# phuang1024/Starst3r

Hardware: AMD Instinct MI355X
Metric: 3DGS train iters/sec @ 1M Gaussians, 8x1080p views (higher is better)
Workload: dtype f32

## Files before the change

starst3r_amd/build.py:

```python
import concurrent.futures as cf
import os
import subprocess
import sys

HERE = os.path.dirname(os.path.abspath(__file__))
CSRC = os.path.join(HERE, "csrc")
OBJ = os.path.join(HERE, "_build")
LIB = os.path.join(HERE, "libst3r_hip.so")
HIPCC = os.environ.get("HIPCC", "/opt/rocm/bin/hipcc")

COMMON = ["--offload-arch=gfx950", "-O3", "-std=c++17", "-fPIC", "-fvisibility=hidden", "-munsafe-fp-atomics",
          "-Wall", "-Wno-unused-function", "-Wno-unused-result", "-DNDEBUG"] + os.environ.get("ST3R_DEFS", "").split()
PER_FILE = {
    "gs_project.hip": ["-ffp-contract=off"],
    "gs_isect.hip": ["-ffp-contract=off"],
    "recip_nn.hip": ["-mllvm", "-amdgpu-mfma-vgpr-form"],
}
NO_PACKED_F32 = ["-Xclang", "-target-feature", "-Xclang", "-packed-fp32-ops"]


def sources():
    return sorted(f for f in os.listdir(CSRC) if f.endswith(".hip"))


def _deps_mtime():
    hdrs = [os.path.join(CSRC, f) for f in os.listdir(CSRC) if f.endswith(".h")]
    hdrs.append(os.path.join(HERE, "..", "include", "st3r.h"))
    return max(os.path.getmtime(h) for h in hdrs)


def _compile(src, force, verbose):
    obj = os.path.join(OBJ, src.replace(".hip", ".o"))
    srcp = os.path.join(CSRC, src)
    if not force and os.path.exists(obj) and os.path.getmtime(obj) > max(os.path.getmtime(srcp), _deps_mtime()):
        return obj, False
    cmd = [HIPCC] + COMMON + NO_PACKED_F32 + PER_FILE.get(src, []) + ["-c", srcp, "-o", obj]
    if verbose:
        print(" ".join(cmd), flush=True)
    r = subprocess.run(cmd, capture_output=True, text=True)
    if r.returncode != 0:
        raise RuntimeError(f"hipcc failed for {src}:\n{r.stdout}\n{r.stderr}")
    noise = "is not a recognized feature for this target"
    err = "\n".join(l for l in r.stderr.splitlines() if l.strip() and noise not in l)
    if verbose and err:
        print(err)
    return obj, True


def build(force=False, verbose=False):
    os.makedirs(OBJ, exist_ok=True)
    srcs = sources()
    with cf.ThreadPoolExecutor(max_workers=min(8, len(srcs))) as ex:
        res = list(ex.map(lambda s: _compile(s, force, verbose), srcs))
    objs = [o for o, _ in res]
    if force or any(c for _, c in res) or not os.path.exists(LIB):
        cmd = [HIPCC, "--offload-arch=gfx950", "-shared", "-fPIC", "-o", LIB] + objs + ["-ldl"]
        if verbose:
            print(" ".join(cmd), flush=True)
        subprocess.check_call(cmd)
    return LIB


if __name__ == "__main__":
    print(build(force="--force" in sys.argv, verbose=("-v" in sys.argv or True)))
```

starst3r_amd/csrc/fused_step.hip:

```cpp
#include "radix_sort.h"
#include "stages.h"

int st3r_count_settle(st3r_ctx* ctx) {
    if (!ctx->count_pending) return ST3R_OK;
    HIP_TRY(hipEventSynchronize(ctx->count_event));
    ctx->count_pending = 0;
    const int64_t n = (int64_t)((int32_t*)(ctx->pinned + 8))[0];
    if (n < 0) {
        ctx->isect_hint = 0;
        ctx->view_chunks = (ctx->view_chunks > 0 ? ctx->view_chunks : 1) * 2;
        st3r_set_error("the previous step produced more than 2^31 tile intersections: its gradients were incomplete -- "
                       "repeat it (st3r_gs_train_fwd_bwd / st3r_gs_train_step now walk the views in %d chunks)",
                       ctx->view_chunks);
        return ST3R_ERR_CAPACITY;
    }
    if (n > ctx->count_cap) {
        ctx->isect_hint = 0;
        st3r_set_error("the previous step produced %lld tile intersections, more than the %lld its buffers were sized "
                       "for from the step before (+25 %%): its gradients were incomplete and st3r_adam_step / "
                       "st3r_gs_train_step did NOT apply them (the update is guarded on the device) -- repeat that step",
                       (long long)n, (long long)ctx->count_cap);
        return ST3R_ERR_CAPACITY;
    }
    ctx->isect_hint = n;
    return ST3R_OK;
}

struct FrontPlan {
    int tile_w, tile_h;
    bool key32;
    bool segments;
    int rect32;
    bool rectbase;
    uint32_t key_base;
    int l1_end_bit;
    int end_bit;
};
static const float k_near_plane = 0.01f, k_far_plane = 1e10f;
static FrontPlan front_plan(int C, int W, int H, int debug_flags, bool with_reg, bool records) {
    FrontPlan p;
    const int tile = 16;
    p.tile_w = (W + tile - 1) / tile; p.tile_h = (H + tile - 1) / tile;
    uint32_t near_bits, far_bits;
    memcpy(&near_bits, &k_near_plane, 4); memcpy(&far_bits, &k_far_plane, 4);
    p.key32 = (C <= 8) && (far_bits - near_bits < 0x1FFFFFFFu);
    p.key_base = p.key32 ? near_bits : 0u;
    p.rect32 = (p.tile_w <= 255 && p.tile_h <= 255 && !(debug_flags & 64)) ? 1 : 0;
    p.segments = p.key32 && with_reg && !records && !(debug_flags & 4);
    p.l1_end_bit = (p.key32 ? 29 : 32) + bit_length_u32((uint32_t)(C - 1));
    p.rectbase = p.tile_w <= 1023 && p.tile_h <= 1023 && !(debug_flags & 64);
    p.end_bit = bit_length_u32((uint32_t)((int64_t)C * p.tile_w * p.tile_h - 1));
    return p;
}

static int rasterize_front(st3r_ctx* ctx, hipStream_t s, const GsParams& g, const GsViews& v, double* reg_sums, int tight,
                           const float* records_in, bool allow_async, RasterOut* o, double* loss_sums = nullptr) {
    const int N = g.N, C = v.C, W = v.W, H = v.H;
    const int tile = 16;
    const FrontPlan fp = front_plan(C, W, H, ctx->debug_flags, reg_sums != nullptr, records_in != nullptr);
    const int tile_w = fp.tile_w, tile_h = fp.tile_h;
    const int64_t n_pairs = (int64_t)N * C;
    float* splats = const_cast<float*>(records_in);
    if (!records_in) {
        ARENA_GET(SLOT_SPLATS, float, n_pairs * ST3R_SPLAT_STRIDE, own);
        splats = own;
    }
    ARENA_GET(SLOT_CUM, int32_t, n_pairs, cum);
    ARENA_GET(SLOT_OFFSETS, int32_t, (int64_t)C * tile_w * tile_h + 1, offsets);
    const float near_plane = k_near_plane, far_plane = k_far_plane;
    const bool key32 = fp.key32;
    ARENA_GET(SLOT_DKEYS_A, uint64_t, n_pairs, dkeys_a);
    ARENA_GET(SLOT_DKEYS_B, uint64_t, n_pairs, dkeys_b);
    ARENA_GET(SLOT_DVALS_A, int32_t, n_pairs, dvals_a);
    ARENA_GET(SLOT_DVALS_B, int32_t, n_pairs, perm);
    const int rect32 = fp.rect32;
    ARENA_GET(SLOT_RECTS, uint64_t, rect32 ? (n_pairs + 1) / 2 : n_pairs, rects);
    int32_t* counts = nullptr;
    { int rc_ = st3r_counts_buffer(ctx, s, &counts); if (rc_) return rc_; }
    uint32_t* const krange = fp.segments ? (uint32_t*)(counts + 8) : nullptr;
    st3r_prof_begin(ctx, s, STG_PROJECT);
    const uint32_t key_base = fp.key_base;
    int rc = records_in
                 ? st3r_records_prepare_impl(s, N, C, splats, tile, tile_w, tile_h, tight, nullptr, dkeys_a, dvals_a,
                                             key_base, rects, rect32)
                 : st3r_project_impl(ctx, s, g, v, tile, 0.3f, near_plane, far_plane, 0.0f, splats, nullptr, reg_sums,
                                     dkeys_a, dvals_a, tight, key_base, rects, rect32, 1, loss_sums, 2 * C, krange);
    if (!rc && records_in && loss_sums) HIP_TRY(hipMemsetAsync(loss_sums, 0, sizeof(double) * 2 * (size_t)C, s));
    st3r_prof_end(ctx, s, STG_PROJECT);
    if (rc) return rc;
    st3r_prof_begin(ctx, s, STG_SORT_DEPTH);
    rc = krange ? st3r_radix_sort_u32_segments(ctx, s, N, C, (uint32_t*)dkeys_a, dvals_a, (uint32_t*)dkeys_b, perm, krange)
         : key32 ? st3r_radix_sort_u32(ctx, s, n_pairs, 0, fp.l1_end_bit, (uint32_t*)dkeys_a, dvals_a, (uint32_t*)dkeys_b, perm, nullptr)
                 : st3r_radix_sort_u64(ctx, s, n_pairs, 0, fp.l1_end_bit, dkeys_a, dvals_a, dkeys_b, perm);
    st3r_prof_end(ctx, s, STG_SORT_DEPTH);
    if (rc) return rc;
    int64_t n_isects = 0;
    st3r_prof_begin(ctx, s, STG_SCAN);
    uint64_t* rectbase = nullptr;
    if (fp.rectbase) {
        ARENA_GET(SLOT_RECTBASE, uint64_t, n_pairs, rb);
        rectbase = rb;
    }
    const int64_t sig = ((int64_t)N << 34) ^ ((int64_t)C << 26) ^ ((int64_t)W << 13) ^ (int64_t)H;
    const bool async = allow_async && ctx->isect_hint > 0 && ctx->hint_sig == sig;
    int32_t* total_dev = nullptr;
    rc = st3r_isect_scan_impl(ctx, s, n_pairs, nullptr, cum, nullptr, rects, rect32, rectbase, &total_dev,
                              async ? counts : nullptr, async ? (int32_t*)(ctx->pinned + 8) : nullptr);
    st3r_prof_end(ctx, s, STG_SCAN);
    if (rc) return rc;
    if (async) {
        if (!ctx->count_event) HIP_TRY(hipEventCreateWithFlags(&ctx->count_event, hipEventDisableTiming));
        HIP_TRY(hipEventRecord(ctx->count_event, s));
        n_isects = ctx->isect_hint + ctx->isect_hint / 4 + 1024;
        if (ctx->debug_flags & 8) n_isects = ctx->isect_hint / 2;
        if (n_isects > 2147483647LL) n_isects = 2147483647LL;
        ctx->count_pending = 1; ctx->count_cap = n_isects;
        o->n_visible = -1; o->n_isects_ref = -1;
    } else {
        HIP_TRY(hipMemcpyAsync(ctx->pinned, total_dev, sizeof(int32_t), hipMemcpyDeviceToHost, s));
        if (reg_sums) HIP_TRY(hipMemcpyAsync(ctx->pinned + 1, reg_sums + 2, 2 * sizeof(double), hipMemcpyDeviceToHost, s));
        HIP_TRY(hipStreamSynchronize(s));
        n_isects = (int64_t)((int32_t*)ctx->pinned)[0];
        if (n_isects < 0) {
            st3r_set_error("more than 2^31 tile intersections in one call: split the views over more calls / GPUs");
            return ST3R_SPLIT_VIEWS;
        }
        o->n_visible = reg_sums ? (int64_t)((double*)ctx->pinned)[1] : -1;
        o->n_isects_ref = reg_sums ? (int64_t)((double*)ctx->pinned)[2] : n_isects;
        if (allow_async) { ctx->isect_hint = n_isects; ctx->hint_sig = sig; }
    }
    ARENA_GET(SLOT_KEYS_A, uint32_t, n_isects, tkeys_a);
    ARENA_GET(SLOT_KEYS_B, uint32_t, n_isects, tkeys_b);
    ARENA_GET(SLOT_VALS_A, int32_t, n_isects, vals_a);
    ARENA_GET(SLOT_VALS_B, int32_t, n_isects, vals_b);
    o->n_records = async ? -1 : n_isects;
    const int64_t n_keys = (int64_t)C * tile_w * tile_h;
    const uint32_t* band_table = nullptr;
    const uint32_t* band_hist = nullptr;
    int n_bands = 0;
    if (n_isects > 0) {
        const int end_bit = fp.end_bit;
        const bool banded = st3r_sort_tile_banded(end_bit, ctx->debug_flags) != 0;
        const bool packed = banded && n_pairs <= (1 << 24) && !(ctx->debug_flags & 1024);
        n_bands = (int)((n_keys - 1) >> 8) + 1;
        st3r_prof_begin(ctx, s, STG_EMIT);
        rc = st3r_isect_emit_chain_impl(ctx, s, N, C, perm, rects, rect32, tile_w, tile_h, packed ? nullptr : tkeys_a, vals_a,
                                        n_isects, banded ? st3r_radix_sort_band_tile(n_isects) : 0, total_dev, &band_table);
        st3r_prof_end(ctx, s, STG_EMIT);
        if (rc) return rc;
        st3r_prof_begin(ctx, s, STG_SORT);
        rc = packed ? st3r_radix_sort_u32_banded_packed(ctx, s, n_isects, n_bands, band_table, (const uint32_t*)vals_a, vals_b,
                                                        &band_hist)
             : banded ? st3r_radix_sort_u32_banded(ctx, s, n_isects, n_bands, band_table, tkeys_a, vals_a, tkeys_b, vals_b)
                      : st3r_sort_tile_impl(ctx, s, n_isects, end_bit, tkeys_a, vals_a, tkeys_b, vals_b, total_dev);
        st3r_prof_end(ctx, s, STG_SORT);
        if (rc) return rc;
    }
    st3r_prof_begin(ctx, s, STG_OFFSETS);
    rc = band_hist ? st3r_radix_band_offsets(s, n_bands, band_table, band_hist, n_keys, offsets)
                   : st3r_isect_offsets32_impl(s, n_isects, tkeys_b, C, tile_w, tile_h, offsets, total_dev);
    st3r_prof_end(ctx, s, STG_OFFSETS);
    if (rc) return rc;
    o->C = C; o->W = W; o->H = H; o->tile_w = tile_w; o->tile_h = tile_h;
    o->splats = splats; o->offsets = offsets; o->flat = vals_b; o->cum = cum; o->rects = rect32 ? nullptr : rects;
    o->rectbase = rectbase;
    o->tight = tight; o->n_pairs = n_pairs;
    o->n_isects = n_isects;
    return ST3R_OK;
}

__global__ void k_finalize_loss(int C, const double* __restrict__ sums, const double* __restrict__ reg_sums,
                                double inv_px, double inv_cnt, double w_l1, double w_ssim, double reg_views,
                                double opac_k, double scale_k, float* __restrict__ loss_out,
                                const double* __restrict__ dsums, const double* __restrict__ dnorm, double depth_fac,
                                const double* __restrict__ wnorm, const double* __restrict__ asums,
                                const double* __restrict__ anorm, double alpha_fac) {
    if (threadIdx.x == 0 && blockIdx.x == 0) {
        double loss = 0;
        if (wnorm)
            for (int c = 0; c < C; ++c)
                loss += w_l1 * sums[2 * c] / (3.0 * fmax(wnorm[2 * c], 1.0)) +
                        w_ssim * (3.0 * wnorm[2 * c + 1] - sums[2 * c + 1]) / (3.0 * fmax(wnorm[2 * c + 1], 1.0));
        else
            for (int c = 0; c < C; ++c) loss += w_l1 * sums[2 * c] * inv_px + w_ssim * (1.0 - sums[2 * c + 1] * inv_cnt);
        loss += reg_views * (opac_k * reg_sums[0] + scale_k * reg_sums[1]);
        if (dsums)
            for (int c = 0; c < C; ++c) loss += depth_fac * dsums[c] / dnorm[c];
        if (asums)
            for (int c = 0; c < C; ++c) loss += alpha_fac * asums[c] / anorm[c];
        loss_out[0] = (float)loss;
    }
}

static int finalize_loss(hipStream_t s, int C, int H, int W, const double* sums, const double* reg_sums, float ssim_fac,
                         double reg_views, double opac_k, double scale_k, float* loss_out, const double* dp_sums,
                         const DepthPrior& dp, const LossWeight& lw, const double* at_sums = nullptr,
                         const AlphaTarget& at = AlphaTarget{}) {
    const int Hi = H - 10, Wi = W - 10;
    const double cnt = (Hi > 0 && Wi > 0) ? (double)Hi * Wi * 3 : 0.0;
    hipLaunchKernelGGL(k_finalize_loss, dim3(1), dim3(64), 0, s, C, sums, reg_sums, 1.0 / ((double)H * W * 3),
                       cnt > 0 ? 1.0 / cnt : 0.0, (double)(1.0f - ssim_fac), (double)ssim_fac, reg_views, opac_k, scale_k,
                       loss_out, dp_sums, dp.norm, (double)dp.fac, lw.weight ? lw.norm : nullptr, at_sums, at.norm,
                       (double)at.fac);
    LAUNCH_CHECK();
    return ST3R_OK;
}

struct LossFacs { float ssim, opac, scale; };

struct ViewBatch {
    GsViews v;
    const float* gt;
    double* sums;
    double* dp_sums;
    float* v_viewmats;
    bool exposure;
    bool weighted;
    bool background;
    double* at_sums;
    ViewBatch slice(int c0, int c1) const {
        return {v.slice(c0, c1), gt + (int64_t)c0 * v.H * v.W * 3, sums + 2 * c0, dp_sums ? dp_sums + c0 : nullptr,
                v_viewmats ? v_viewmats + 16 * c0 : nullptr, exposure, weighted, background,
                at_sums ? at_sums + c0 : nullptr};
    }
};

struct StepImages { float *rgb, *alpha; int32_t* last; float *v_rgb, *depth, *v_depth, *v_alpha, *exposed, *composite; };

static int step_images(st3r_ctx* ctx, const RasterOut& ro, bool with_depth, bool with_exposure, bool with_background,
                       bool with_v_alpha, StepImages* im) {
    const int64_t n_px = (int64_t)ro.C * ro.H * ro.W;
    ARENA_GET(SLOT_RGB, float, n_px * 3, rgb);
    ARENA_GET(SLOT_ALPHA, float, n_px, alpha);
    ARENA_GET(SLOT_LAST, int32_t, n_px, last);
    ARENA_GET(SLOT_VRENDER, float, n_px * 3, v_rgb);
    *im = StepImages{rgb, alpha, last, v_rgb, nullptr, nullptr, nullptr, nullptr, nullptr};
    if (with_exposure) {
        ARENA_GET(SLOT_EXPOSED, float, n_px * 3, exposed);
        im->exposed = exposed;
    }
    if (with_background) {
        ARENA_GET(SLOT_COMPOSITE, float, n_px * 3, composite);
        im->composite = composite;
    }
    if (with_depth) {
        ARENA_GET(SLOT_DEPTH, float, n_px, depth);
        ARENA_GET(SLOT_VDEPTH, float, n_px, v_depth);
        im->depth = depth; im->v_depth = v_depth;
    }
    if (with_depth || with_v_alpha) {
        ARENA_GET(SLOT_VALPHA, float, n_px, v_alpha);
        im->v_alpha = v_alpha;
    }
    return ST3R_OK;
}

static int forward_and_losses(st3r_ctx* ctx, hipStream_t s, const RasterOut& ro, const ViewBatch& b, float ssim_fac,
                              bool sums_cleared, const DepthPrior& dp, const ExposureReg& ex, const LossWeight& lw,
                              const StepImages& im, const Background& bg = Background{},
                              const AlphaTarget& at = AlphaTarget{}) {
    const bool eio = true;
    st3r_prof_begin(ctx, s, STG_BLEND_FWD);
    int rc = st3r_blend_fwd_impl(ctx, s, ro, im.rgb, im.alpha, im.last, true, eio);
    if (!rc && dp.prior) rc = st3r_blend_depth_fwd_impl(ctx, s, ro, im.last, im.depth, eio);
    st3r_prof_end(ctx, s, STG_BLEND_FWD);
    if (rc) return rc;
    st3r_prof_begin(ctx, s, STG_LOSS);
    const float* x = im.rgb;
    if (bg.colors) {
        rc = st3r_composite_fwd_impl(s, ro.C, ro.H, ro.W, im.rgb, im.alpha, bg.colors, im.composite);
        x = im.composite;
    }
    if (!rc && ex.exposure) rc = st3r_exposure_fwd_impl(s, ro.C, ro.H, ro.W, x, ex.exposure, im.exposed);
    if (!rc)
        rc = st3r_loss_impl(ctx, s, ro.C, ro.H, ro.W, ex.exposure ? im.exposed : x, b.gt, 1.0f - ssim_fac, ssim_fac,
                            b.sums, im.v_rgb, sums_cleared, lw);
    if (!rc && ex.exposure)
        rc = st3r_exposure_bwd_impl(ctx, s, ro.C, ro.H, ro.W, x, ex.exposure, im.v_rgb, im.v_rgb, ex.v_exposure);
    if (!rc && dp.prior)
        rc = st3r_depth_prior_loss_impl(ctx, s, ro.C, ro.H, ro.W, im.depth, im.alpha, dp.prior, dp.weight, dp.norm, 1, dp.fac,
                                        b.dp_sums, 1, im.v_depth, im.v_alpha);
    if (!rc && (bg.colors || at.target))
        rc = st3r_alpha_grad_impl(ctx, s, ro.C, ro.H, ro.W, im.alpha, bg.colors, bg.colors ? im.v_rgb : nullptr, at.target,
                                  at.weight, at.norm, 1, at.fac, dp.prior ? im.v_alpha : nullptr, b.at_sums, 1, im.v_alpha,
                                  nullptr);
    st3r_prof_end(ctx, s, STG_LOSS);
    return rc;
}

static int blend_backward(st3r_ctx* ctx, hipStream_t s, const RasterOut& ro, const StepImages& im, bool need_pairs,
                          st3r_vtile_ref* slots, float* v_pairs) {
    RasterOut rb = ro;
    if (ctx->debug_flags & 2) { rb.rects = nullptr; rb.rectbase = nullptr; }
    const bool eio = true;
    st3r_prof_begin(ctx, s, STG_BLEND_BWD);
    int rc = st3r_blend_bwd_impl(ctx, s, rb, im.alpha, im.last, im.v_rgb, im.v_alpha, nullptr, eio, slots);
    if (!rc && need_pairs) {
        ARENA_GET(SLOT_VSPLATS_D, float, ro.n_pairs * ST3R_SPLAT_STRIDE, v_pairs_d);
        rc = st3r_blend_depth_bwd_impl(ctx, s, rb, im.alpha, im.last, im.v_depth, v_pairs_d, eio);
        if (!rc) {
            if (slots->vtile) rc = st3r_gather_vtile_impl(s, ro.n_pairs, slots, v_pairs);
            else HIP_TRY(hipMemsetAsync(v_pairs, 0, sizeof(float) * ST3R_SPLAT_STRIDE * (size_t)ro.n_pairs, s));
        }
        if (!rc) rc = st3r_add_pairs_impl(s, ro.n_pairs, v_pairs, v_pairs_d);
    }
    st3r_prof_end(ctx, s, STG_BLEND_BWD);
    return rc;
}

static int project_backward(st3r_ctx* ctx, hipStream_t s, const GsParams& g, const GsViews& v, const RasterOut& ro,
                            const LossFacs& f, const float* v_pairs, const st3r_vtile_ref* slots, bool accumulate,
                            float* grads) {
    ctx->ranges_recorded = 0;
    if (!(ctx->n_ranges > 1 && ctx->comm_stream))
        return st3r_project_sh_bwd_impl(s, g, v, 0.3f, ro.splats, v_pairs, (float)v.C, f.opac, f.scale, grads, accumulate, 0,
                                        -1, false, slots);
    ARENA_GET(SLOT_GSTAGE, float, (int64_t)23 * g.N, gstage);
    const int K = ctx->n_ranges;
    for (int j = 0; j < K; ++j) {
        const int g0 = (int)((int64_t)g.N * j / K), g1 = (int)((int64_t)g.N * (j + 1) / K);
        int rc = st3r_project_sh_bwd_impl(s, g, v, 0.3f, ro.splats, v_pairs, (float)v.C, f.opac, f.scale, gstage, accumulate,
                                          g0, g1, true, slots);
        if (rc) return rc;
        HIP_TRY(hipEventRecord(ctx->ev_range_bwd[j], s));
    }
    ctx->ranges_recorded = K;
    return ST3R_OK;
}

static int pose_backward(st3r_ctx* ctx, hipStream_t s, const GsParams& g, const GsViews& v, const RasterOut& ro,
                         const float* v_pairs, float* v_viewmats) {
    return st3r_gs_viewmat_bwd(ctx, s, g.N, v.C, g.means, g.quats, g.scales, g.sh, g.sh_stride, v.viewmats, v.Ks, v.campos,
                               v.W, v.H, 0.3f, ro.splats, v_pairs, v_viewmats);
}

static int train_views(st3r_ctx* ctx, hipStream_t s, const GsParams& g, const ViewBatch& b, const LossFacs& f,
                       double* reg_sums, bool allow_async, bool accumulate, float* grads, RasterOut* ro_out) {
    const GsViews& v = b.v;
    DepthPrior dp{};
    int rc = b.dp_sums ? st3r_depth_prior_for(ctx, s, b.gt, v.C, v.H, v.W, &dp) : ST3R_OK;
    if (rc) return rc;
    ExposureReg ex{};
    if (b.exposure) st3r_exposure_for(ctx, b.gt, v.C, v.H, v.W, &ex);
    LossWeight lw{};
    if (b.weighted) rc = st3r_loss_weight_for(ctx, s, b.gt, v.C, v.H, v.W, &lw);
    if (rc) return rc;
    Background bg{};
    if (b.background) st3r_background_for(ctx, b.gt, v.C, v.H, v.W, &bg);
    AlphaTarget at{};
    if (b.at_sums) rc = st3r_alpha_target_for(ctx, s, b.gt, v.C, v.H, v.W, &at);
    if (rc) return rc;
    const bool need_pairs = dp.prior != nullptr;
    RasterOut& ro = *ro_out;
    rc = rasterize_front(ctx, s, g, v, reg_sums, 1, nullptr, allow_async, &ro, b.sums);
    if (rc) return rc;
    StepImages im;
    rc = step_images(ctx, ro, need_pairs, ex.exposure != nullptr, bg.colors != nullptr, bg.colors || at.target, &im);
    if (rc) return rc;
    float* const v_Ks = st3r_intrinsics_grad_for(ctx, b.gt, v.C, v.H, v.W);
    float* v_pairs = nullptr;
    if (need_pairs || b.v_viewmats || v_Ks) {
        ARENA_GET(SLOT_VSPLATS, float, ro.n_pairs * ST3R_SPLAT_STRIDE, vp);
        v_pairs = vp;
    }
    rc = forward_and_losses(ctx, s, ro, b, f.ssim, true, dp, ex, lw, im, bg, at);
    if (rc) return rc;
    st3r_vtile_ref slots{};
    rc = blend_backward(ctx, s, ro, im, need_pairs, &slots, v_pairs);
    if (rc) return rc;
    st3r_prof_begin(ctx, s, STG_PROJECT_BWD);
    rc = project_backward(ctx, s, g, v, ro, f, need_pairs ? v_pairs : nullptr, need_pairs ? nullptr : &slots, accumulate,
                          grads);
    if (!rc && need_pairs && b.v_viewmats) rc = pose_backward(ctx, s, g, v, ro, v_pairs, b.v_viewmats);
    if (!rc && need_pairs) rc = st3r_gs_depth_bwd(ctx, s, g.N, v.C, g.means, v.viewmats, ro.splats, v_pairs, grads, b.v_viewmats);
    st3r_prof_end(ctx, s, STG_PROJECT_BWD);
    if (!rc && !need_pairs && (b.v_viewmats || v_Ks)) {
        rc = st3r_gather_vtile_impl(s, ro.n_pairs, &slots, v_pairs);
        if (!rc && b.v_viewmats) rc = pose_backward(ctx, s, g, v, ro, v_pairs, b.v_viewmats);
    }
    if (!rc && v_Ks)
        rc = st3r_gs_intrinsics_bwd(ctx, s, g.N, v.C, g.means, g.quats, g.scales, v.viewmats, v.Ks, v.W, v.H, 0.3f,
                                    ro.splats, v_pairs, v_Ks);
    return rc;
}

static int train_chunks(st3r_ctx* ctx, hipStream_t s, const GsParams& g, const ViewBatch& all, const LossFacs& f,
                        double* reg_sums, double* reg_scratch, bool want_stats, float* grads, int* chunks, int64_t stats[3]) {
    const int C = all.v.C;
    for (;;) {
        int rc = ST3R_OK;
        stats[0] = stats[1] = stats[2] = 0;
        bool first = true;
        for (int k = 0; k < *chunks && !rc; ++k) {
            const int c0 = (int)((int64_t)k * C / *chunks), c1 = (int)((int64_t)(k + 1) * C / *chunks);
            if (c1 == c0) continue;
            RasterOut ro;
            rc = train_views(ctx, s, g, all.slice(c0, c1), f, first ? reg_sums : reg_scratch,
                             !want_stats && *chunks == 1 && !ctx->comm, !first, grads, &ro);
            if (!rc) { stats[0] += ro.n_visible; stats[1] += ro.n_records; stats[2] += ro.n_isects_ref; }
            first = false;
        }
        if (rc == ST3R_SPLIT_VIEWS && *chunks < C) {
            *chunks = *chunks * 2 < C ? *chunks * 2 : C;
            continue;
        }
        return rc == ST3R_SPLIT_VIEWS ? ST3R_ERR_INVALID : rc;
    }
}

int st3r_train_fwd_bwd_impl(st3r_ctx* ctx, hipStream_t s, const GsParams& g, const GsViews& v, const float* gt_images,
                            float ssim_fac, float opac_fac, float scale_fac, float* grads, float* loss_out,
                            int64_t* stats_host, float* v_viewmats) {
    const int N = g.N, C = v.C;
    ARG_CHECK(ctx && N > 0 && C > 0 && C <= ST3R_MAX_VIEWS && v.W > 0 && v.H > 0 && g.sh_stride >= 12);
    ARG_CHECK((int64_t)N * C < 2147483647LL);
    ARG_CHECK(g.means && g.quats && g.scales && g.opacities && g.sh && v.viewmats && v.Ks && v.campos && gt_images && grads &&
              loss_out);
    ARENA_GET(SLOT_SMALL, double, 2 * (size_t)C + 12, small);
    double* sums = small;
    double* reg_sums = small + 2 * C;
    double* dp_sums = nullptr;
    DepthPrior dp;
    int rc = st3r_depth_prior_for(ctx, s, gt_images, C, v.H, v.W, &dp);
    if (rc) return rc;
    if (dp.prior) {
        if (ctx->comm) {
            st3r_set_error("a depth prior is registered and a communicator is attached -- the depth term is not "
                           "supported in view-sharded training (clear it with st3r_ctx_set_depth_prior(ctx, NULL, ...))");
            return ST3R_ERR_INVALID;
        }
        ARENA_GET(SLOT_DPRIOR_SUMS, double, (size_t)C, ds);
        dp_sums = ds;
    }
    ExposureReg ex;
    st3r_exposure_for(ctx, gt_images, C, v.H, v.W, &ex);
    if (ex.exposure && ctx->comm) {
        st3r_set_error("exposures are registered and a communicator is attached -- per-view exposures are not supported "
                       "in view-sharded training (clear them with st3r_ctx_set_exposure(ctx, NULL, ...))");
        return ST3R_ERR_INVALID;
    }
    if (ctx->comm && st3r_intrinsics_grad_for(ctx, gt_images, C, v.H, v.W)) {
        st3r_set_error("an intrinsics gradient is registered and a communicator is attached -- intrinsics refinement is "
                       "not supported in view-sharded training (clear it with st3r_ctx_set_intrinsics_grad(ctx, NULL, ...))");
        return ST3R_ERR_INVALID;
    }
    LossWeight lw;
    rc = st3r_loss_weight_for(ctx, s, gt_images, C, v.H, v.W, &lw);
    if (rc) return rc;
    if (lw.weight && ctx->comm) {
        st3r_set_error("loss weights are registered and a communicator is attached -- per-pixel loss weights are not "
                       "supported in view-sharded training (clear them with st3r_ctx_set_loss_weight(ctx, NULL, ...))");
        return ST3R_ERR_INVALID;
    }
    Background bg;
    st3r_background_for(ctx, gt_images, C, v.H, v.W, &bg);
    if (bg.colors && ctx->comm) {
        st3r_set_error("backgrounds are registered and a communicator is attached -- backgrounds are not supported in "
                       "view-sharded training (clear them with st3r_ctx_set_background(ctx, NULL, ...))");
        return ST3R_ERR_INVALID;
    }
    double* at_sums = nullptr;
    AlphaTarget at;
    rc = st3r_alpha_target_for(ctx, s, gt_images, C, v.H, v.W, &at);
    if (rc) return rc;
    if (at.target) {
        if (ctx->comm) {
            st3r_set_error("alpha targets are registered and a communicator is attached -- alpha supervision is not "
                           "supported in view-sharded training (clear them with st3r_ctx_set_alpha_target(ctx, NULL, ...))");
            return ST3R_ERR_INVALID;
        }
        ARENA_GET(SLOT_ATARGET_SUMS, double, (size_t)C, as);
        at_sums = as;
    }
    st3r_prof_next_step(ctx);
    rc = st3r_count_settle(ctx);
    if (rc) return rc;
    int chunks = ctx->view_chunks > 0 ? ctx->view_chunks : 1;
    if ((ctx->debug_flags & 32) && chunks < 2) chunks = 2;
    if (chunks > C) chunks = C;
    int64_t stats[3];
    rc = train_chunks(ctx, s, g, ViewBatch{v, gt_images, sums, dp_sums, v_viewmats, ex.exposure != nullptr, lw.weight != nullptr,
                                           bg.colors != nullptr, at_sums},
                      LossFacs{ssim_fac, opac_fac, scale_fac},
                      reg_sums, reg_sums + 4, stats_host != nullptr, grads, &chunks, stats);
    if (rc) return rc;
    if (chunks > 1) ctx->view_chunks = chunks;
    rc = finalize_loss(s, C, v.H, v.W, sums, reg_sums, ssim_fac, (double)C, (double)opac_fac / N,
                       (double)scale_fac / (3.0 * N), loss_out, dp_sums, dp, lw, at_sums, at);
    if (rc) return rc;
    if (stats_host) {
        stats_host[0] = stats[0]; stats_host[1] = stats[1]; stats_host[2] = st3r_ctx_arena_bytes(ctx);
        stats_host[3] = stats[2];
    }
    return ST3R_OK;
}

ST3R_EXPORT int st3r_gs_train_fwd_bwd(st3r_ctx* ctx, void* stream, int N, int C, const float* means,
                                      const float* quats, const float* scales, const float* opacities,
                                      const float* sh, int sh_stride, const float* viewmats, const float* Ks,
                                      const float* campos, const float* gt_images, int width, int height,
                                      float ssim_fac, float opac_fac, float scale_fac, float* grads,
                                      float* loss_out, int64_t* stats_host) {
    return st3r_train_fwd_bwd_impl(ctx, (hipStream_t)stream, GsParams{N, means, quats, scales, opacities, sh, sh_stride},
                                   GsViews{C, width, height, viewmats, Ks, campos}, gt_images, ssim_fac, opac_fac,
                                   scale_fac, grads, loss_out, stats_host, nullptr);
}

ST3R_EXPORT int st3r_gs_raster_train(st3r_ctx* ctx, void* stream, int N, int C, const float* records,
                                     const float* gt_images, int width, int height, float ssim_fac,
                                     float* v_records, float* loss_out, int64_t* stats_host) {
    ARG_CHECK(ctx && N > 0 && C > 0 && width > 0 && height > 0 && records && gt_images && v_records && loss_out);
    ARG_CHECK(C <= ST3R_MAX_VIEWS && (int64_t)N * C < 2147483647LL);
    hipStream_t s = (hipStream_t)stream;
    ARENA_GET(SLOT_SMALL, double, 2 * (size_t)C + 8, sums);
    double* reg_sums = sums + 2 * C;
    const ViewBatch b{GsViews{C, width, height}, gt_images, sums, nullptr, nullptr, false, false, false, nullptr};
    HIP_TRY(hipMemsetAsync(reg_sums, 0, sizeof(double) * 4, s));
    st3r_prof_next_step(ctx);
    RasterOut ro;
    int rc = st3r_count_settle(ctx);
    if (rc) return rc;
    rc = rasterize_front(ctx, s, GsParams{N}, b.v, nullptr, 1, records, stats_host == nullptr, &ro);
    if (rc == ST3R_SPLIT_VIEWS) rc = ST3R_ERR_INVALID;
    if (rc) return rc;
    StepImages im;
    rc = step_images(ctx, ro, false, false, false, false, &im);
    if (rc) return rc;
    rc = forward_and_losses(ctx, s, ro, b, ssim_fac, false, DepthPrior{}, ExposureReg{}, LossWeight{}, im);
    if (rc) return rc;
    st3r_prof_begin(ctx, s, STG_BLEND_BWD);
    rc = st3r_blend_bwd_impl(ctx, s, ro, im.alpha, im.last, im.v_rgb, nullptr, v_records, true, nullptr);
    st3r_prof_end(ctx, s, STG_BLEND_BWD);
    if (rc) return rc;
    rc = finalize_loss(s, C, height, width, sums, reg_sums, ssim_fac, 0.0, 0.0, 0.0, loss_out, nullptr, DepthPrior{},
                       LossWeight{});
    if (rc) return rc;
    if (stats_host) {
        stats_host[0] = -1; stats_host[1] = ro.n_records; stats_host[2] = st3r_ctx_arena_bytes(ctx); stats_host[3] = -1;
    }
    return ST3R_OK;
}

ST3R_EXPORT int st3r_gs_render(st3r_ctx* ctx, void* stream, int N, int C, const float* means, const float* quats,
                               const float* scales, const float* opacities, const float* sh, int sh_stride,
                               const float* viewmats, const float* Ks, const float* campos, int width, int height,
                               float* rgb, float* alpha, int64_t* stats_host) {
    ARG_CHECK(ctx && N > 0 && C > 0 && width > 0 && height > 0 && sh_stride >= 12);
    ARG_CHECK(C <= ST3R_MAX_VIEWS && (int64_t)N * C < 2147483647LL);
    ARG_CHECK(means && quats && scales && opacities && sh && viewmats && Ks && campos && rgb && alpha);
    hipStream_t s = (hipStream_t)stream;
    RasterOut ro;
    int rc = st3r_count_settle(ctx);
    if (rc) return rc;
    rc = rasterize_front(ctx, s, GsParams{N, means, quats, scales, opacities, sh, sh_stride},
                         GsViews{C, width, height, viewmats, Ks, campos}, nullptr, 0, nullptr, false, &ro);
    if (rc == ST3R_SPLIT_VIEWS) rc = ST3R_ERR_INVALID;
    if (rc) return rc;
    ARENA_GET(SLOT_LAST, int32_t, (int64_t)C * height * width, last);
    rc = st3r_blend_fwd_impl(ctx, s, ro, rgb, alpha, last, false, true);
    if (rc) return rc;
    if (stats_host) {
        stats_host[0] = -1; stats_host[1] = ro.n_records; stats_host[2] = st3r_ctx_arena_bytes(ctx); stats_host[3] = 0;
    }
    return ST3R_OK;
}

ST3R_EXPORT int st3r_front_plan(int N, int C, int width, int height, int debug_flags, int training, int records,
                                int64_t n_records, int64_t* out, int n_out) {
    ARG_CHECK(N > 0 && C > 0 && C <= ST3R_MAX_VIEWS && width > 0 && height > 0 && n_records >= 0 && out &&
              n_out >= ST3R_FRONT_PLAN_WORDS && !(training && records));
    const FrontPlan fp = front_plan(C, width, height, debug_flags, training != 0, records != 0);
    const int64_t n_pairs = (int64_t)N * C;
    for (int i = 0; i < n_out; ++i) out[i] = 0;
    out[0] = fp.rect32; out[1] = fp.rectbase; out[2] = fp.key32; out[3] = fp.segments;
    out[4] = st3r_scan_tiles(n_pairs);
    int bpc, grid, self_base;
    st3r_emit_grid(N, C, &bpc, &grid, &self_base);
    out[5] = bpc; out[6] = grid; out[7] = self_base;
    int64_t sh[8];
    if (fp.segments) st3r_radix_sort_shape(4, n_pairs, N, C, 0, 0, sh);
    else st3r_radix_sort_shape(fp.key32 ? 4 : 8, n_pairs, 0, 0, 0, fp.l1_end_bit, sh);
    out[8] = sh[0]; out[9] = sh[1]; out[10] = sh[2]; out[11] = sh[3]; out[12] = sh[4];
    out[25] = sh[5];
    out[fp.key32 ? 26 : 28] = sh[6]; out[fp.key32 ? 27 : 29] = sh[7];
    st3r_radix_sort_shape(fp.key32 ? 8 : 4, 1, 0, 0, 0, 8, sh);
    out[fp.key32 ? 28 : 26] = sh[6]; out[fp.key32 ? 29 : 27] = sh[7];
    out[13] = st3r_sort_tile_end_bit(fp.end_bit);
    if (n_records > 0) {
        st3r_radix_sort_shape(4, n_records, 0, 0, 0, (int)out[13], sh);
        out[14] = sh[0]; out[15] = sh[1]; out[16] = sh[2]; out[17] = sh[4];
    }
    if (st3r_sort_tile_banded(fp.end_bit, debug_flags)) {
        out[18] = 1;
        out[19] = (((int64_t)C * fp.tile_w * fp.tile_h - 1) >> 8) + 1;
        if (n_records > 0) out[30] = n_records / st3r_radix_sort_band_tile(n_records) + out[19];
    }
    int64_t k[5];
    st3r_isect_constants(k);
    for (int i = 0; i < 5; ++i) out[20 + i] = k[i];
    return ST3R_OK;
}
```

starst3r_amd/csrc/gs_intrinsics.hip:

```cpp
#include "per_view.h"
#include "project_common.h"

__global__ __launch_bounds__(256) void k_intrinsics_bwd_part(
    int N, const float* __restrict__ means, const float* __restrict__ quats, const float* __restrict__ scales,
    const float* __restrict__ viewmats, const float* __restrict__ Ks, int W, int H, const float4* __restrict__ splats,
    const float4* __restrict__ v_splats, double* __restrict__ part) {
    __shared__ double red[4 * 4];
    const int c = blockIdx.y;
    const int g = blockIdx.x * blockDim.x + threadIdx.x;
    float v_fx = 0.f, v_fy = 0.f, v_cx = 0.f, v_cy = 0.f;
    const int64_t pid = (int64_t)c * N + g;
    if (g < N && __float_as_int(splats[pid * 3 + 2].z) > 0) {
        const float4 r0 = splats[pid * 3 + 0], r1 = splats[pid * 3 + 1];
        const float4 g0 = v_splats[pid * 3 + 0], g1 = v_splats[pid * 3 + 1];
        const float* V = viewmats + 16 * c;
        const float R[9] = {V[0], V[1], V[2], V[4], V[5], V[6], V[8], V[9], V[10]};
        const float* K = Ks + 9 * c;
        const float fx = K[0], fy = K[4], cx = K[2], cy = K[5];
        const float tan_fovx = 0.5f * (float)W / fx, tan_fovy = 0.5f * (float)H / fy;
        const float lim_xp = ((float)W - cx) / fx + 0.3f * tan_fovx, lim_xn = cx / fx + 0.3f * tan_fovx;
        const float lim_yp = ((float)H - cy) / fy + 0.3f * tan_fovy, lim_yn = cy / fy + 0.3f * tan_fovy;
        const float mx = means[3 * g], my = means[3 * g + 1], mz = means[3 * g + 2];
        float qw = quats[4 * g], qx = quats[4 * g + 1], qy = quats[4 * g + 2], qz = quats[4 * g + 3];
        const float sc[3] = {scales[3 * g], scales[3 * g + 1], scales[3 * g + 2]};
        const float inv_norm = 1.0f / sqrtf(((qw * qw + qx * qx) + qy * qy) + qz * qz);
        qw *= inv_norm; qx *= inv_norm; qy *= inv_norm; qz *= inv_norm;
        float cov[6];
        {
            float x2 = qx * qx, y2 = qy * qy, z2 = qz * qz, xy = qx * qy, xz = qx * qz, yz = qy * qz;
            float wx = qw * qx, wy = qw * qy, wz = qw * qz;
            const float Rq[9] = {1.0f - 2.0f * (y2 + z2), 2.0f * (xy - wz), 2.0f * (xz + wy),
                                 2.0f * (xy + wz), 1.0f - 2.0f * (x2 + z2), 2.0f * (yz - wx),
                                 2.0f * (xz - wy), 2.0f * (yz + wx), 1.0f - 2.0f * (x2 + y2)};
            float M[9];
#pragma unroll
            for (int i = 0; i < 3; ++i)
#pragma unroll
                for (int j = 0; j < 3; ++j) M[i * 3 + j] = Rq[i * 3 + j] * sc[j];
            cov[0] = M[0] * M[0] + M[1] * M[1] + M[2] * M[2];
            cov[1] = M[0] * M[3] + M[1] * M[4] + M[2] * M[5];
            cov[2] = M[0] * M[6] + M[1] * M[7] + M[2] * M[8];
            cov[3] = M[3] * M[3] + M[4] * M[4] + M[5] * M[5];
            cov[4] = M[3] * M[6] + M[4] * M[7] + M[5] * M[8];
            cov[5] = M[6] * M[6] + M[7] * M[7] + M[8] * M[8];
        }
        const float x = R[0] * mx + R[1] * my + R[2] * mz + V[3];
        const float y = R[3] * mx + R[4] * my + R[5] * mz + V[7];
        const float z = R[6] * mx + R[7] * my + R[8] * mz + V[11];
        float T[9];
#pragma unroll
        for (int i = 0; i < 3; ++i) {
            T[i * 3 + 0] = R[i * 3] * cov[0] + R[i * 3 + 1] * cov[1] + R[i * 3 + 2] * cov[2];
            T[i * 3 + 1] = R[i * 3] * cov[1] + R[i * 3 + 1] * cov[3] + R[i * 3 + 2] * cov[4];
            T[i * 3 + 2] = R[i * 3] * cov[2] + R[i * 3 + 1] * cov[4] + R[i * 3 + 2] * cov[5];
        }
        const Sym3 S = {T[0] * R[0] + T[1] * R[1] + T[2] * R[2], T[0] * R[3] + T[1] * R[4] + T[2] * R[5],
                        T[0] * R[6] + T[1] * R[7] + T[2] * R[8], T[3] * R[3] + T[4] * R[4] + T[5] * R[5],
                        T[3] * R[6] + T[4] * R[7] + T[5] * R[8], T[6] * R[6] + T[7] * R[7] + T[8] * R[8]};
        const float rz = 1.0f / z, rz2 = rz * rz;
        const float xr = x * rz, yr = y * rz;
        const bool x_in = (xr <= lim_xp) && (xr >= -lim_xn);
        const bool y_in = (yr <= lim_yp) && (yr >= -lim_yn);
        const float tx = z * fminf(lim_xp, fmaxf(-lim_xn, xr));
        const float ty = z * fminf(lim_yp, fmaxf(-lim_yn, yr));
        const float a = fx * rz, cj = -fx * tx * rz2, b = fy * rz, d = -fy * ty * rz2;
        Sym3 vS;
        float vJ00, vJ02, vJ11, vJ12;
        conic_chain(r0, r1, g0, g1, a, cj, b, d, S, vS, vJ00, vJ02, vJ11, vJ12);
        const float vm2x = g0.x, vm2y = g0.y;
        v_fx = vm2x * xr + vJ00 * rz;
        v_fy = vm2y * yr + vJ11 * rz;
        v_cx = vm2x; v_cy = vm2y;
        if (x_in) v_fx += -x * rz2 * vJ02;
        else v_cx += vJ02 * rz;
        if (y_in) v_fy += -y * rz2 * vJ12;
        else v_cy += vJ12 * rz;
    }
    double v[4] = {(double)v_fx, (double)v_fy, (double)v_cx, (double)v_cy};
    const double t = block_sum_fixed(v, red);
    if (threadIdx.x < 4) part[((int64_t)c * gridDim.x + blockIdx.x) * 4 + threadIdx.x] = t;
}

ST3R_EXPORT int st3r_gs_intrinsics_bwd(st3r_ctx* ctx, void* stream, int N, int C, const float* means, const float* quats,
                                       const float* scales, const float* viewmats, const float* Ks, int width, int height,
                                       float eps2d, const float* splats, const float* v_splats, float* v_Ks) {
    ARG_CHECK(ctx && N >= 0 && C > 0 && C <= ST3R_MAX_VIEWS && width > 0 && height > 0);
    ARG_CHECK(means && quats && scales && viewmats && Ks && splats && v_splats && v_Ks);
    (void)eps2d;
    hipStream_t s = (hipStream_t)stream;
    const int nb = ceil_div(N, 256);
    double* part = nullptr;
    if (nb > 0) {
        ARENA_GET(SLOT_KGRAD_PART, double, 4 * (size_t)nb * C, p);
        part = p;
        hipLaunchKernelGGL(k_intrinsics_bwd_part, dim3(nb, C), dim3(256), 0, s, N, means, quats, scales, viewmats, Ks,
                           width, height, (const float4*)splats, (const float4*)v_splats, part);
        LAUNCH_CHECK();
    }
    return stream_finish<4>(s, C, nb, (const double*)part, v_Ks, 4, 0);
}

float* st3r_intrinsics_grad_for(st3r_ctx* ctx, const float* gt, int C, int H, int W) {
    const int64_t c0 = view_reg_first(ctx->kg, gt, C, H, W);
    return c0 < 0 ? nullptr : ctx->kg_v_Ks + 4 * c0;
}

ST3R_EXPORT int st3r_ctx_set_intrinsics_grad(st3r_ctx* ctx, const float* gt, float* v_Ks, int C, int height, int width) {
    ARG_CHECK(ctx);
    const bool on = gt && v_Ks;
    int rc = view_reg_set(&ctx->kg, on, gt, C, height, width);
    if (rc) return rc;
    ctx->kg_v_Ks = on ? v_Ks : nullptr;
    return ST3R_OK;
}

__global__ __launch_bounds__(64) void k_intrinsics_adam(int C, PerViewAdamK k, float* __restrict__ Ks,
                                                        const float* __restrict__ v_Ks, float* __restrict__ k_m,
                                                        float* __restrict__ k_v, double W, double H, int mode) {
    const int c = per_view_adam_view(k, C);
    if (c < 0) return;
    float* K = Ks + 9 * c;
    const float* G = v_Ks + 4 * c;
    float* m = k_m + 4 * c;
    float* v = k_v + 4 * c;
    const double fx = (double)K[0], fy = (double)K[4];
    const double g0 = fx * (double)G[0], g1 = fy * (double)G[1];
    if (mode & 1) {
        const double e = exp(per_view_adam_delta<false>(k, m[0], g0 + g1, v[0]));
        K[0] = (float)(fx * e); K[4] = (float)(fy * e);
    } else {
        K[0] = (float)(fx * exp(per_view_adam_delta<false>(k, m[0], g0, v[0])));
        K[4] = (float)(fy * exp(per_view_adam_delta<false>(k, m[1], g1, v[1])));
    }
    if (mode & 2) {
        K[2] = (float)((double)K[2] + W * per_view_adam_delta<false>(k, m[2], W * (double)G[2], v[2]));
        K[5] = (float)((double)K[5] + H * per_view_adam_delta<false>(k, m[3], H * (double)G[3], v[3]));
    }
}

ST3R_EXPORT int st3r_intrinsics_adam_step(st3r_ctx* ctx, void* stream, int C, float* Ks, const float* v_Ks, float* k_m,
                                          float* k_v, double lr, double beta1, double beta2, double eps, int step,
                                          const float* mask, int width, int height, int mode) {
    ARG_CHECK(ctx && C > 0 && step >= 1 && beta1 >= 0.0 && beta1 < 1.0 && beta2 >= 0.0 && beta2 < 1.0);
    ARG_CHECK(Ks && v_Ks && k_m && k_v && width > 0 && height > 0 && mode >= 0 && mode <= 3);
    return per_view_adam_launch(ctx, (hipStream_t)stream, k_intrinsics_adam, C, lr, beta1, beta2, eps, step, mask, Ks, v_Ks,
                                k_m, k_v, (double)width, (double)height, mode);
}
```

starst3r_amd/csrc/gs_pose_bwd.hip:

```cpp
#include "per_view.h"
#include "project_common.h"

#define POSE_VALS 15

__device__ __forceinline__ void block_sum_pose(double (&v)[POSE_VALS], double* red) {
    const double sum = block_sum_fixed(v, red);
    if (threadIdx.x < POSE_VALS) red[4 * POSE_VALS + threadIdx.x] = sum;
    __syncthreads();
    if (threadIdx.x < POSE_VALS) red[threadIdx.x] = red[4 * POSE_VALS + threadIdx.x];
    __syncthreads();
}

__global__ __launch_bounds__(256) void k_viewmat_bwd_part(
    int N, const float* __restrict__ means, const float* __restrict__ quats, const float* __restrict__ scales,
    const float* __restrict__ sh, int sh_stride, const float* __restrict__ viewmats, const float* __restrict__ Ks,
    const float* __restrict__ campos, int W, int H, const float4* __restrict__ splats,
    const float4* __restrict__ v_splats, double* __restrict__ part) {
    __shared__ double red[5 * POSE_VALS];
    const int c = blockIdx.y;
    const int g = blockIdx.x * blockDim.x + threadIdx.x;
    float acc[POSE_VALS];
#pragma unroll
    for (int k = 0; k < POSE_VALS; ++k) acc[k] = 0.f;
    const int64_t pid = (int64_t)c * N + g;
    if (g < N && __float_as_int(splats[pid * 3 + 2].z) > 0) {
        const float4 r0 = splats[pid * 3 + 0], r1 = splats[pid * 3 + 1], r2 = splats[pid * 3 + 2];
        const float4 g0 = v_splats[pid * 3 + 0], g1 = v_splats[pid * 3 + 1], g2 = v_splats[pid * 3 + 2];
        const float* V = viewmats + 16 * c;
        const float R[9] = {V[0], V[1], V[2], V[4], V[5], V[6], V[8], V[9], V[10]};
        const float* K = Ks + 9 * c;
        const float fx = K[0], fy = K[4], cx = K[2], cy = K[5];
        const float tan_fovx = 0.5f * (float)W / fx, tan_fovy = 0.5f * (float)H / fy;
        const float lim_xp = ((float)W - cx) / fx + 0.3f * tan_fovx, lim_xn = cx / fx + 0.3f * tan_fovx;
        const float lim_yp = ((float)H - cy) / fy + 0.3f * tan_fovy, lim_yn = cy / fy + 0.3f * tan_fovy;
        const float mx = means[3 * g], my = means[3 * g + 1], mz = means[3 * g + 2];
        float qw = quats[4 * g], qx = quats[4 * g + 1], qy = quats[4 * g + 2], qz = quats[4 * g + 3];
        const float sc[3] = {scales[3 * g], scales[3 * g + 1], scales[3 * g + 2]};
        float k[12];
        const float* kp = sh + (int64_t)g * sh_stride;
#pragma unroll
        for (int i = 0; i < 12; ++i) k[i] = kp[i];
        const float inv_norm = 1.0f / sqrtf(((qw * qw + qx * qx) + qy * qy) + qz * qz);
        qw *= inv_norm; qx *= inv_norm; qy *= inv_norm; qz *= inv_norm;
        float cov[6];
        {
            float x2 = qx * qx, y2 = qy * qy, z2 = qz * qz, xy = qx * qy, xz = qx * qz, yz = qy * qz;
            float wx = qw * qx, wy = qw * qy, wz = qw * qz;
            const float Rq[9] = {1.0f - 2.0f * (y2 + z2), 2.0f * (xy - wz), 2.0f * (xz + wy),
                                 2.0f * (xy + wz), 1.0f - 2.0f * (x2 + z2), 2.0f * (yz - wx),
                                 2.0f * (xz - wy), 2.0f * (yz + wx), 1.0f - 2.0f * (x2 + y2)};
            float M[9];
#pragma unroll
            for (int i = 0; i < 3; ++i)
#pragma unroll
                for (int j = 0; j < 3; ++j) M[i * 3 + j] = Rq[i * 3 + j] * sc[j];
            cov[0] = M[0] * M[0] + M[1] * M[1] + M[2] * M[2];
            cov[1] = M[0] * M[3] + M[1] * M[4] + M[2] * M[5];
            cov[2] = M[0] * M[6] + M[1] * M[7] + M[2] * M[8];
            cov[3] = M[3] * M[3] + M[4] * M[4] + M[5] * M[5];
            cov[4] = M[3] * M[6] + M[4] * M[7] + M[5] * M[8];
            cov[5] = M[6] * M[6] + M[7] * M[7] + M[8] * M[8];
        }
        {
            float dx = mx - campos[3 * c], dy = my - campos[3 * c + 1], dz = mz - campos[3 * c + 2];
            float nrm = sqrtf(dx * dx + dy * dy + dz * dz);
            float inrm = 1.0f / nrm;
            float ux = dx * inrm, uy = dy * inrm, uz = dz * inrm;
            const float vcol[3] = {g1.z, g1.w, g2.x};
            const float colf[3] = {r1.z, r1.w, r2.x};
            float vdx = 0.f, vdy = 0.f, vdz = 0.f;
#pragma unroll
            for (int ch = 0; ch < 3; ++ch) {
                float pre = SH_C0 * k[ch] + SH_C1 * ((-uy * k[3 + ch] + uz * k[6 + ch]) - ux * k[9 + ch]) + 0.5f;
                float vc = (colf[ch] > 0.0f || pre >= 0.0f) ? vcol[ch] : 0.0f;
                vdx += -SH_C1 * k[9 + ch] * vc;
                vdy += -SH_C1 * k[3 + ch] * vc;
                vdz += SH_C1 * k[6 + ch] * vc;
            }
            float dotp = vdx * ux + vdy * uy + vdz * uz;
            acc[12] = -((vdx - dotp * ux) * inrm);
            acc[13] = -((vdy - dotp * uy) * inrm);
            acc[14] = -((vdz - dotp * uz) * inrm);
        }
        const float x = R[0] * mx + R[1] * my + R[2] * mz + V[3];
        const float y = R[3] * mx + R[4] * my + R[5] * mz + V[7];
        const float z = R[6] * mx + R[7] * my + R[8] * mz + V[11];
        float T[9];
#pragma unroll
        for (int i = 0; i < 3; ++i) {
            T[i * 3 + 0] = R[i * 3] * cov[0] + R[i * 3 + 1] * cov[1] + R[i * 3 + 2] * cov[2];
            T[i * 3 + 1] = R[i * 3] * cov[1] + R[i * 3 + 1] * cov[3] + R[i * 3 + 2] * cov[4];
            T[i * 3 + 2] = R[i * 3] * cov[2] + R[i * 3 + 1] * cov[4] + R[i * 3 + 2] * cov[5];
        }
        const float S00 = T[0] * R[0] + T[1] * R[1] + T[2] * R[2];
        const float S01 = T[0] * R[3] + T[1] * R[4] + T[2] * R[5];
        const float S02 = T[0] * R[6] + T[1] * R[7] + T[2] * R[8];
        const float S11 = T[3] * R[3] + T[4] * R[4] + T[5] * R[5];
        const float S12 = T[3] * R[6] + T[4] * R[7] + T[5] * R[8];
        const float S22 = T[6] * R[6] + T[7] * R[7] + T[8] * R[8];
        const float rz = 1.0f / z, rz2 = rz * rz, rz3 = rz2 * rz;
        const float xr = x * rz, yr = y * rz;
        const bool x_in = (xr <= lim_xp) && (xr >= -lim_xn);
        const bool y_in = (yr <= lim_yp) && (yr >= -lim_yn);
        const float tx = z * fminf(lim_xp, fmaxf(-lim_xn, xr));
        const float ty = z * fminf(lim_yp, fmaxf(-lim_yn, yr));
        const float a = fx * rz, cj = -fx * tx * rz2, b = fy * rz, d = -fy * ty * rz2;
        const Sym3 S = {S00, S01, S02, S11, S12, S22};
        Sym3 vS;
        float vJ00, vJ02, vJ11, vJ12;
        conic_chain(r0, r1, g0, g1, a, cj, b, d, S, vS, vJ00, vJ02, vJ11, vJ12);
        const float vm2x = g0.x, vm2y = g0.y;
        float vpx = fx * rz * vm2x;
        float vpy = fy * rz * vm2y;
        float vpz = -(fx * x * vm2x + fy * y * vm2y) * rz2;
        vpz += -fx * rz2 * vJ00 - fy * rz2 * vJ11;
        if (x_in) { vpx += -fx * rz2 * vJ02; vpz += 2.0f * fx * x * rz3 * vJ02; }
        else { vpz += fx * tx * rz3 * vJ02; }
        if (y_in) { vpy += -fy * rz2 * vJ12; vpz += 2.0f * fy * y * rz3 * vJ12; }
        else { vpz += fy * ty * rz3 * vJ12; }
        const float vSm[9] = {vS.xx, vS.xy, vS.xz, vS.xy, vS.yy, vS.yz, vS.xz, vS.yz, vS.zz};
        const float vp[3] = {vpx, vpy, vpz}, m[3] = {mx, my, mz};
#pragma unroll
        for (int i = 0; i < 3; ++i) {
#pragma unroll
            for (int j = 0; j < 3; ++j)
                acc[i * 3 + j] = vp[i] * m[j] +
                                 2.0f * (vSm[i * 3] * T[j] + vSm[i * 3 + 1] * T[3 + j] + vSm[i * 3 + 2] * T[6 + j]);
            acc[9 + i] = vp[i];
        }
    }
    double v[POSE_VALS];
#pragma unroll
    for (int k2 = 0; k2 < POSE_VALS; ++k2) v[k2] = (double)acc[k2];
    block_sum_pose(v, red);
    if (threadIdx.x < POSE_VALS)
        part[((int64_t)c * gridDim.x + blockIdx.x) * POSE_VALS + threadIdx.x] = red[threadIdx.x];
}

__global__ __launch_bounds__(256) void k_viewmat_bwd_finish(int n_part, const float* __restrict__ viewmats,
                                                           const double* __restrict__ part,
                                                           float* __restrict__ v_viewmats) {
    __shared__ double red[5 * POSE_VALS];
    const int c = blockIdx.x;
    double v[POSE_VALS];
#pragma unroll
    for (int k = 0; k < POSE_VALS; ++k) v[k] = 0.0;
    const double* pc = part + (int64_t)c * n_part * POSE_VALS;
    for (int b = threadIdx.x; b < n_part; b += blockDim.x) {
#pragma unroll
        for (int k = 0; k < POSE_VALS; ++k) v[k] += pc[(int64_t)b * POSE_VALS + k];
    }
    block_sum_pose(v, red);
    if (threadIdx.x >= 16) return;
    double a[16];
    const float* Vf = viewmats + 16 * c;
#pragma unroll
    for (int i = 0; i < 16; ++i) a[i] = (double)Vf[i];
    const double s0 = a[0] * a[5] - a[4] * a[1], s1 = a[0] * a[6] - a[4] * a[2], s2 = a[0] * a[7] - a[4] * a[3];
    const double s3 = a[1] * a[6] - a[5] * a[2], s4 = a[1] * a[7] - a[5] * a[3], s5 = a[2] * a[7] - a[6] * a[3];
    const double c5 = a[10] * a[15] - a[14] * a[11], c4 = a[9] * a[15] - a[13] * a[11], c3 = a[9] * a[14] - a[13] * a[10];
    const double c2 = a[8] * a[15] - a[12] * a[11], c1 = a[8] * a[14] - a[12] * a[10], c0 = a[8] * a[13] - a[12] * a[9];
    const double idet = 1.0 / (s0 * c5 - s1 * c4 + s2 * c3 + s3 * c2 - s4 * c1 + s5 * c0);
    double inv[16];
    inv[0] = (a[5] * c5 - a[6] * c4 + a[7] * c3) * idet;
    inv[1] = (-a[1] * c5 + a[2] * c4 - a[3] * c3) * idet;
    inv[2] = (a[13] * s5 - a[14] * s4 + a[15] * s3) * idet;
    inv[3] = (-a[9] * s5 + a[10] * s4 - a[11] * s3) * idet;
    inv[4] = (-a[4] * c5 + a[6] * c2 - a[7] * c1) * idet;
    inv[5] = (a[0] * c5 - a[2] * c2 + a[3] * c1) * idet;
    inv[6] = (-a[12] * s5 + a[14] * s2 - a[15] * s1) * idet;
    inv[7] = (a[8] * s5 - a[10] * s2 + a[11] * s1) * idet;
    inv[8] = (a[4] * c4 - a[5] * c2 + a[7] * c0) * idet;
    inv[9] = (-a[0] * c4 + a[1] * c2 - a[3] * c0) * idet;
    inv[10] = (a[12] * s4 - a[13] * s2 + a[15] * s0) * idet;
    inv[11] = (-a[8] * s4 + a[9] * s2 - a[11] * s0) * idet;
    inv[12] = (-a[4] * c3 + a[5] * c1 - a[6] * c0) * idet;
    inv[13] = (a[0] * c3 - a[1] * c1 + a[2] * c0) * idet;
    inv[14] = (-a[12] * s3 + a[13] * s1 - a[14] * s0) * idet;
    inv[15] = (a[8] * s3 - a[9] * s1 + a[10] * s0) * idet;
    const int i = threadIdx.x >> 2, j = threadIdx.x & 3;
    const double u = inv[i] * red[12] + inv[4 + i] * red[13] + inv[8 + i] * red[14];
    const double w = inv[4 * j + 3];
    const double base = i == 3 ? 0.0 : (j == 3 ? red[9 + i] : red[i * 3 + j]);
    v_viewmats[16 * c + threadIdx.x] = (float)(base - u * w);
}

ST3R_EXPORT int st3r_gs_viewmat_bwd(st3r_ctx* ctx, void* stream, int N, int C, const float* means, const float* quats,
                                    const float* scales, const float* sh, int sh_stride, const float* viewmats,
                                    const float* Ks, const float* campos, int width, int height, float eps2d,
                                    const float* splats, const float* v_splats, float* v_viewmats) {
    ARG_CHECK(ctx && N >= 0 && C > 0 && C <= ST3R_MAX_VIEWS && sh_stride >= 12 && width > 0 && height > 0);
    ARG_CHECK(means && quats && scales && sh && viewmats && Ks && campos && splats && v_splats && v_viewmats);
    (void)eps2d;
    hipStream_t s = (hipStream_t)stream;
    const int nb = ceil_div(N, 256);
    double* part = nullptr;
    if (nb > 0) {
        ARENA_GET(SLOT_POSE_PART, double, POSE_VALS * (size_t)nb * C, p);
        part = p;
        hipLaunchKernelGGL(k_viewmat_bwd_part, dim3(nb, C), dim3(256), 0, s, N, means, quats, scales, sh, sh_stride,
                           viewmats, Ks, campos, width, height, (const float4*)splats, (const float4*)v_splats, part);
        LAUNCH_CHECK();
    }
    hipLaunchKernelGGL(k_viewmat_bwd_finish, dim3(C), dim3(256), 0, s, nb, viewmats, (const double*)part, v_viewmats);
    LAUNCH_CHECK();
    return ST3R_OK;
}
```

starst3r_amd/csrc/gs_project.hip:

```cpp
#include "stages.h"
#include "tile_rect.h"
#include "project_common.h"

__device__ __forceinline__ float dot3f(float a0, float a1, float a2, float b0, float b1, float b2) {
    return (a0 * b0 + a1 * b1) + a2 * b2;
}

__global__ __launch_bounds__(256) void k_project_sh_fwd(
    int N, int C, const float* __restrict__ means, const float* __restrict__ quats,
    const float* __restrict__ scales, const float* __restrict__ opacities, const float* __restrict__ sh,
    int sh_stride, const float* __restrict__ viewmats, const float* __restrict__ Ks,
    const float* __restrict__ campos, int W, int H, int tile_size, int tile_w, int tile_h, float eps2d,
    float near_plane, float far_plane, float radius_clip, float4* __restrict__ splats,
    int32_t* __restrict__ tiles_per_gauss, double* __restrict__ reg_part,
    uint64_t* __restrict__ depth_keys, int32_t* __restrict__ depth_vals, int tight, uint32_t key_base,
    void* __restrict__ rects, int rect32, uint32_t* __restrict__ krange_part) {
    extern __shared__ float cam[];
    __shared__ float red[8];
    for (int c = threadIdx.x; c < C; c += blockDim.x) {
        float* o = cam + c * CAM_STRIDE;
        const float* V = viewmats + 16 * c;
        for (int k = 0; k < 12; ++k) o[k] = V[k];
        const float* K = Ks + 9 * c;
        float fx = K[0], fy = K[4], cx = K[2], cy = K[5];
        o[12] = fx; o[13] = fy; o[14] = cx; o[15] = cy;
        float tan_fovx = 0.5f * (float)W / fx;
        float tan_fovy = 0.5f * (float)H / fy;
        o[16] = ((float)W - cx) / fx + 0.3f * tan_fovx;
        o[17] = cx / fx + 0.3f * tan_fovx;
        o[18] = ((float)H - cy) / fy + 0.3f * tan_fovy;
        o[19] = cy / fy + 0.3f * tan_fovy;
        o[20] = campos[3 * c]; o[21] = campos[3 * c + 1]; o[22] = campos[3 * c + 2];
    }
    __syncthreads();

    const int g = blockIdx.x * blockDim.x + threadIdx.x;
    const bool active = g < N;
    float mx = 0, my = 0, mz = 0, opac = 0;
    float cov0 = 0, cov1 = 0, cov2 = 0, cov3 = 0, cov4 = 0, cov5 = 0;
    float k[12];
    float reg_o = 0.f, reg_s = 0.f;
    if (active) {
        mx = means[3 * g]; my = means[3 * g + 1]; mz = means[3 * g + 2];
        opac = opacities[g];
        float qw = quats[4 * g], qx = quats[4 * g + 1], qy = quats[4 * g + 2], qz = quats[4 * g + 3];
        float s0 = scales[3 * g], s1 = scales[3 * g + 1], s2 = scales[3 * g + 2];
        const float* kp = sh + (int64_t)g * sh_stride;
#pragma unroll
        for (int i = 0; i < 12; ++i) k[i] = kp[i];
        float n2 = ((qw * qw + qx * qx) + qy * qy) + qz * qz;
        float inv = 1.0f / sqrtf(n2);
        qw *= inv; qx *= inv; qy *= inv; qz *= inv;
        float x2 = qx * qx, y2 = qy * qy, z2 = qz * qz;
        float xy = qx * qy, xz = qx * qz, yz = qy * qz;
        float wx = qw * qx, wy = qw * qy, wz = qw * qz;
        float m0 = (1.0f - 2.0f * (y2 + z2)) * s0, m1 = (2.0f * (xy - wz)) * s1, m2 = (2.0f * (xz + wy)) * s2;
        float m3 = (2.0f * (xy + wz)) * s0, m4 = (1.0f - 2.0f * (x2 + z2)) * s1, m5 = (2.0f * (yz - wx)) * s2;
        float m6 = (2.0f * (xz - wy)) * s0, m7 = (2.0f * (yz + wx)) * s1, m8 = (1.0f - 2.0f * (x2 + y2)) * s2;
        cov0 = dot3f(m0, m1, m2, m0, m1, m2);
        cov1 = dot3f(m0, m1, m2, m3, m4, m5);
        cov2 = dot3f(m0, m1, m2, m6, m7, m8);
        cov3 = dot3f(m3, m4, m5, m3, m4, m5);
        cov4 = dot3f(m3, m4, m5, m6, m7, m8);
        cov5 = dot3f(m6, m7, m8, m6, m7, m8);
        if (reg_part) {
            reg_o = 1.0f / (1.0f + __expf(-opac));
            reg_s = (__expf(s0) + __expf(s1)) + __expf(s2);
        }
    }
    if (reg_part) {
        for (int off = 32; off > 0; off >>= 1) {
            reg_o += __shfl_down(reg_o, off);
            reg_s += __shfl_down(reg_s, off);
        }
        int w = threadIdx.x >> 6;
        if ((threadIdx.x & 63) == 0) { red[w] = reg_o; red[4 + w] = reg_s; }
        __syncthreads();
        if (threadIdx.x == 0) {
            reg_part[4 * blockIdx.x + 0] = (double)((red[0] + red[1]) + (red[2] + red[3]));
            reg_part[4 * blockIdx.x + 1] = (double)((red[4] + red[5]) + (red[6] + red[7]));
        }
    }
    int n_vis = 0, n_ref = 0;
    uint32_t kmin = 0xFFFFFFFFu, kmax = 0u;
    for (int c = 0; active && c < C; ++c) {
        const float* o = cam + c * CAM_STRIDE;
        const float R00 = o[0], R01 = o[1], R02 = o[2], t0 = o[3];
        const float R10 = o[4], R11 = o[5], R12 = o[6], t1 = o[7];
        const float R20 = o[8], R21 = o[9], R22 = o[10], t2 = o[11];
        const int64_t pid = (int64_t)c * N + g;
        float x = dot3f(R00, R01, R02, mx, my, mz) + t0;
        float y = dot3f(R10, R11, R12, mx, my, mz) + t1;
        float z = dot3f(R20, R21, R22, mx, my, mz) + t2;
        bool valid = !(z < near_plane || z > far_plane);
        float m2x = 0, m2y = 0, ca = 0, cb = 0, cc = 0, radius = 0;
        if (valid) {
            float T0 = dot3f(R00, R01, R02, cov0, cov1, cov2), T1 = dot3f(R00, R01, R02, cov1, cov3, cov4),
                  T2 = dot3f(R00, R01, R02, cov2, cov4, cov5);
            float T3 = dot3f(R10, R11, R12, cov0, cov1, cov2), T4 = dot3f(R10, R11, R12, cov1, cov3, cov4),
                  T5 = dot3f(R10, R11, R12, cov2, cov4, cov5);
            float T6 = dot3f(R20, R21, R22, cov0, cov1, cov2), T7 = dot3f(R20, R21, R22, cov1, cov3, cov4),
                  T8 = dot3f(R20, R21, R22, cov2, cov4, cov5);
            float c0 = dot3f(T0, T1, T2, R00, R01, R02);
            float c1 = dot3f(T0, T1, T2, R10, R11, R12);
            float c2 = dot3f(T0, T1, T2, R20, R21, R22);
            float c3 = dot3f(T3, T4, T5, R10, R11, R12);
            float c4 = dot3f(T3, T4, T5, R20, R21, R22);
            float c5 = dot3f(T6, T7, T8, R20, R21, R22);
            const float fx = o[12], fy = o[13], cx = o[14], cy = o[15];
            float rz = 1.0f / z;
            float rz2 = rz * rz;
            float xr = x * rz, yr = y * rz;
            float tx = z * fminf(o[16], fmaxf(-o[17], xr));
            float ty = z * fminf(o[18], fmaxf(-o[19], yr));
            float a = fx * rz, cj = -(fx * tx) * rz2;
            float b = fy * rz, d = -(fy * ty) * rz2;
            float t0x = a * c0 + cj * c2;
            float t0y = a * c1 + cj * c4;
            float t0z = a * c2 + cj * c5;
            float t1y = b * c3 + d * c4;
            float t1z = b * c4 + d * c5;
            float c00 = t0x * a + t0z * cj;
            float c01 = t0y * b + t0z * d;
            float c11 = t1y * b + t1z * d;
            m2x = (fx * x) * rz + cx;
            m2y = (fy * y) * rz + cy;
            c00 += eps2d; c11 += eps2d;
            float det = c00 * c11 - c01 * c01;
            if (det <= 0.0f) valid = false;
            else {
                float inv_det = 1.0f / det;
                ca = c11 * inv_det; cb = -c01 * inv_det; cc = c00 * inv_det;
                float bb = 0.5f * (c00 + c11);
                float v1 = bb + sqrtf(fmaxf(0.01f, bb * bb - det));
                radius = ceilf(3.0f * sqrtf(v1));
                if (radius <= radius_clip) valid = false;
                else if (m2x + radius <= 0.0f || m2x - radius >= (float)W || m2y + radius <= 0.0f ||
                         m2y - radius >= (float)H)
                    valid = false;
            }
        }
        float4 r0 = make_float4(0, 0, 0, 0), r1 = r0, r2 = r0;
        int ntiles = 0;
        TileRect tr = {0, 0, 0, 0};
        if (valid) {
            float dx = mx - o[20], dy = my - o[21], dz = mz - o[22];
            float inorm = 1.0f / sqrtf((dx * dx + dy * dy) + dz * dz);
            dx *= inorm; dy *= inorm; dz *= inorm;
            float col[3];
#pragma unroll
            for (int ch = 0; ch < 3; ++ch) {
                float r = SH_C0 * k[ch];
                r = r + SH_C1 * ((-dy * k[3 + ch] + dz * k[6 + ch]) - dx * k[9 + ch]);
                r = r + 0.5f;
                col[ch] = r < 0.0f ? 0.0f : r;
            }
            tr = ref_tile_rect(m2x, m2y, radius, tile_size, tile_w, tile_h);
            n_ref += (tr.y1 - tr.y0) * (tr.x1 - tr.x0);
            if (tight) tr = tight_tile_rect(tr, m2x, m2y, opac, ca, cb, cc);
            ntiles = (tr.y1 - tr.y0) * (tr.x1 - tr.x0);
            r0 = make_float4(m2x, m2y, opac, ca);
            r1 = make_float4(cb, cc, col[0], col[1]);
            r2 = make_float4(col[2], z, __int_as_float((int)radius), 0.0f);
        }
        splats[pid * 3 + 0] = r0;
        splats[pid * 3 + 1] = r1;
        splats[pid * 3 + 2] = r2;
        if (tiles_per_gauss) tiles_per_gauss[pid] = ntiles;
        if (rects) rect_store(rects, rect32, pid, tr);
        if (depth_keys) {
            const uint32_t dbits = valid ? (uint32_t)__float_as_int(z) : 0xFFFFFFFFu;
            if (key_base) {
                const uint32_t kk = valid ? dbits - key_base : 0x1FFFFFFFu;
                reinterpret_cast<uint32_t*>(depth_keys)[pid] = (krange_part ? 0u : ((uint32_t)c << 29)) | kk;
                if (valid) { kmin = min(kmin, kk); kmax = max(kmax, kk); }
            } else
                depth_keys[pid] = ((uint64_t)c << 32) | dbits;
            if (!krange_part) depth_vals[pid] = (int32_t)pid;
        }
        n_vis += valid ? 1 : 0;
    }
    if (krange_part) {
        for (int off = 32; off > 0; off >>= 1) { kmin = min(kmin, (uint32_t)__shfl_down((int)kmin, off)); kmax = max(kmax, (uint32_t)__shfl_down((int)kmax, off)); }
        __shared__ uint32_t redk[8];
        const int w = threadIdx.x >> 6;
        if ((threadIdx.x & 63) == 0) { redk[w] = kmin; redk[4 + w] = kmax; }
        __syncthreads();
        if (threadIdx.x == 0) {
            krange_part[2 * blockIdx.x + 0] = min(min(redk[0], redk[1]), min(redk[2], redk[3]));
            krange_part[2 * blockIdx.x + 1] = max(max(redk[4], redk[5]), max(redk[6], redk[7]));
        }
    }
    if (reg_part) {
        for (int off = 32; off > 0; off >>= 1) { n_vis += __shfl_down(n_vis, off); n_ref += __shfl_down(n_ref, off); }
        __shared__ int redi[8];
        const int w = threadIdx.x >> 6;
        if ((threadIdx.x & 63) == 0) { redi[w] = n_vis; redi[4 + w] = n_ref; }
        __syncthreads();
        if (threadIdx.x == 0) {
            reg_part[4 * blockIdx.x + 2] = (double)((redi[0] + redi[1]) + (redi[2] + redi[3]));
            reg_part[4 * blockIdx.x + 3] = (double)((redi[4] + redi[5]) + (redi[6] + redi[7]));
        }
    }
}

__global__ __launch_bounds__(256) void k_reg_reduce(int n_blocks, const double* __restrict__ reg_part,
                                                    double* __restrict__ reg_sums, int overwrite,
                                                    double* __restrict__ zero_ptr, int zero_n,
                                                    const uint32_t* __restrict__ krange_part,
                                                    uint32_t* __restrict__ krange) {
    for (int i = threadIdx.x; i < zero_n; i += 256) zero_ptr[i] = 0.0;
    if (krange_part) {
        __shared__ uint32_t shk[2][256];
        uint32_t lo = 0xFFFFFFFFu, hi = 0u;
        for (int b = threadIdx.x; b < n_blocks; b += 256) { lo = min(lo, krange_part[2 * b]); hi = max(hi, krange_part[2 * b + 1]); }
        shk[0][threadIdx.x] = lo; shk[1][threadIdx.x] = hi;
        __syncthreads();
        for (int off = 128; off > 0; off >>= 1) {
            if (threadIdx.x < off) {
                shk[0][threadIdx.x] = min(shk[0][threadIdx.x], shk[0][threadIdx.x + off]);
                shk[1][threadIdx.x] = max(shk[1][threadIdx.x], shk[1][threadIdx.x + off]);
            }
            __syncthreads();
        }
        if (threadIdx.x == 0) {
            lo = shk[0][0]; hi = shk[1][0];
            if (hi < lo) { lo = 0u; hi = 0u; }
            const uint32_t top = hi - lo + 1u;
            krange[0] = lo; krange[1] = top;
            krange[2] = top < (1u << 8) ? 1u : top < (1u << 16) ? 2u : top < (1u << 24) ? 3u : 4u;
        }
        __syncthreads();
    }
    __shared__ double sh[4][256];
    double acc[4] = {0, 0, 0, 0};
    for (int b = threadIdx.x; b < n_blocks; b += 256)
        for (int k = 0; k < 4; ++k) acc[k] += reg_part[4 * b + k];
    for (int k = 0; k < 4; ++k) sh[k][threadIdx.x] = acc[k];
    __syncthreads();
    for (int off = 128; off > 0; off >>= 1) {
        if (threadIdx.x < off)
            for (int k = 0; k < 4; ++k) sh[k][threadIdx.x] += sh[k][threadIdx.x + off];
        __syncthreads();
    }
    if (threadIdx.x < 4) reg_sums[threadIdx.x] = (overwrite ? 0.0 : reg_sums[threadIdx.x]) + sh[threadIdx.x][0];
}

int st3r_project_impl(st3r_ctx* ctx, hipStream_t s, const GsParams& g, const GsViews& v, int tile_size, float eps2d,
                      float near_plane, float far_plane, float radius_clip, float* splats, int32_t* tiles_per_gauss,
                      double* reg_sums, uint64_t* depth_keys, int32_t* depth_vals, int tight, uint32_t key_base, void* rects,
                      int rect32, int reg_overwrite, double* zero_ptr, int zero_n, uint32_t* krange) {
    const int N = g.N, C = v.C, width = v.W, height = v.H;
    if (N == 0) {
        if (reg_sums && reg_overwrite) HIP_TRY(hipMemsetAsync(reg_sums, 0, sizeof(double) * 4, s));
        if (zero_ptr && zero_n > 0) HIP_TRY(hipMemsetAsync(zero_ptr, 0, sizeof(double) * (size_t)zero_n, s));
        return ST3R_OK;
    }
    int tile_w = (width + tile_size - 1) / tile_size, tile_h = (height + tile_size - 1) / tile_size;
    dim3 grid(ceil_div(N, 256)), block(256);
    size_t shmem = (size_t)C * CAM_STRIDE * sizeof(float);
    double* reg_part = nullptr;
    if (reg_sums) {
        ARENA_GET(SLOT_REG_PART, double, 4 * (size_t)grid.x, p);
        reg_part = p;
    }
    uint32_t* krange_part = nullptr;
    if (krange && reg_sums) {
        ARENA_GET(SLOT_KRANGE_PART, uint32_t, 2 * (size_t)grid.x, p);
        krange_part = p;
    }
    hipLaunchKernelGGL(k_project_sh_fwd, grid, block, shmem, s, N, C, g.means, g.quats, g.scales, g.opacities, g.sh,
                       g.sh_stride, v.viewmats, v.Ks, v.campos, width, height, tile_size, tile_w, tile_h, eps2d, near_plane, far_plane,
                       radius_clip, (float4*)splats, tiles_per_gauss, reg_part, depth_keys, depth_vals, tight, key_base,
                       rects, rect32, krange_part);
    if (reg_sums)
        hipLaunchKernelGGL(k_reg_reduce, dim3(1), dim3(256), 0, s, (int)grid.x, reg_part, reg_sums, reg_overwrite, zero_ptr,
                           zero_ptr ? zero_n : 0, (const uint32_t*)krange_part, krange);
    else if (zero_ptr && zero_n > 0)
        HIP_TRY(hipMemsetAsync(zero_ptr, 0, sizeof(double) * (size_t)zero_n, s));
    LAUNCH_CHECK();
    return ST3R_OK;
}

ST3R_EXPORT int st3r_gs_project_sh(st3r_ctx* ctx, void* stream, int N, int C, const float* means,
                                   const float* quats, const float* scales, const float* opacities,
                                   const float* sh, int sh_stride, const float* viewmats, const float* Ks,
                                   const float* campos, int width, int height, int tile_size, float eps2d,
                                   float near_plane, float far_plane, float radius_clip, float* splats,
                                   int32_t* tiles_per_gauss, double* reg_sums) {
    ARG_CHECK(ctx && N >= 0 && C > 0 && C <= ST3R_MAX_VIEWS && sh_stride >= 12 && width > 0 && height > 0 && tile_size > 0);
    ARG_CHECK(means && quats && scales && opacities && sh && viewmats && Ks && campos && splats && tiles_per_gauss);
    return st3r_project_impl(ctx, (hipStream_t)stream, GsParams{N, means, quats, scales, opacities, sh, sh_stride},
                             GsViews{C, width, height, viewmats, Ks, campos}, tile_size, eps2d, near_plane, far_plane, radius_clip, splats,
                             tiles_per_gauss, reg_sums, nullptr, nullptr, 0, 0u, nullptr, 0, 0, nullptr, 0, nullptr);
}
```

starst3r_amd/csrc/gs_project_bwd.hip:

```cpp
#include "stages.h"
#include "blend_common.h"
#include "project_common.h"

#ifndef GATHER_WIDE_ABOVE
#define GATHER_WIDE_ABOVE 6
#endif

template <bool GATHER>
__global__ __launch_bounds__(256) __attribute__((amdgpu_waves_per_eu(4))) void k_project_sh_bwd(
    int N, int C, const float* __restrict__ means, const float* __restrict__ quats,
    const float* __restrict__ scales, const float* __restrict__ opacities, const float* __restrict__ sh,
    int sh_stride, const float* __restrict__ viewmats, const float* __restrict__ Ks,
    const float* __restrict__ campos, int W, int H, float eps2d, const float4* __restrict__ splats,
    const float4* __restrict__ v_splats, float reg_o_k, float reg_s_k, float* __restrict__ grads, int accumulate,
    int g_begin, int g_end, int range_major, const int32_t* __restrict__ cum, const float* __restrict__ vtile, int stamp,
    unsigned vt_cap, const uint32_t* __restrict__ touch) {
    extern __shared__ float cam[];
    constexpr int ROW = ACC_VALS;
    __shared__ float sVal[GATHER ? 256 * ROW : 1];
    __shared__ float sAcc[GATHER ? 256 * ROW : 1];
    __shared__ int sStart[GATHER ? 4 * 65 : 1];
    for (int c = threadIdx.x; c < C; c += blockDim.x) {
        float* o = cam + c * CAM_STRIDE;
        const float* V = viewmats + 16 * c;
        for (int k = 0; k < 12; ++k) o[k] = V[k];
        const float* K = Ks + 9 * c;
        float fx = K[0], fy = K[4], cx = K[2], cy = K[5];
        o[12] = fx; o[13] = fy; o[14] = cx; o[15] = cy;
        float tan_fovx = 0.5f * (float)W / fx;
        float tan_fovy = 0.5f * (float)H / fy;
        o[16] = ((float)W - cx) / fx + 0.3f * tan_fovx;
        o[17] = cx / fx + 0.3f * tan_fovx;
        o[18] = ((float)H - cy) / fy + 0.3f * tan_fovy;
        o[19] = cy / fy + 0.3f * tan_fovy;
        o[20] = campos[3 * c]; o[21] = campos[3 * c + 1]; o[22] = campos[3 * c + 2];
    }
    __syncthreads();
    const int gbase = g_begin + blockIdx.x * blockDim.x;
    const bool valid = gbase + (int)threadIdx.x < g_end;
    if (!GATHER && !valid) return;
    const int g = valid ? gbase + (int)threadIdx.x : g_end - 1;

    const float mx = means[3 * g], my = means[3 * g + 1], mz = means[3 * g + 2];
    const float opac = opacities[g];
    float qw = quats[4 * g], qx = quats[4 * g + 1], qy = quats[4 * g + 2], qz = quats[4 * g + 3];
    const float s0 = scales[3 * g], s1 = scales[3 * g + 1], s2 = scales[3 * g + 2];
    float k[12];
    const float* kp = sh + (int64_t)g * sh_stride;
#pragma unroll
    for (int i = 0; i < 12; ++i) k[i] = kp[i];
    const float inv_norm = 1.0f / sqrtf(((qw * qw + qx * qx) + qy * qy) + qz * qz);
    qw *= inv_norm; qx *= inv_norm; qy *= inv_norm; qz *= inv_norm;
    const float sc[3] = {s0, s1, s2};
    auto rot_and_m = [&](float (&Rq)[9], float (&M)[9]) {
        float x2 = qx * qx, y2 = qy * qy, z2 = qz * qz, xy = qx * qy, xz = qx * qz, yz = qy * qz;
        float wx = qw * qx, wy = qw * qy, wz = qw * qz;
        Rq[0] = 1.0f - 2.0f * (y2 + z2); Rq[1] = 2.0f * (xy - wz); Rq[2] = 2.0f * (xz + wy);
        Rq[3] = 2.0f * (xy + wz); Rq[4] = 1.0f - 2.0f * (x2 + z2); Rq[5] = 2.0f * (yz - wx);
        Rq[6] = 2.0f * (xz - wy); Rq[7] = 2.0f * (yz + wx); Rq[8] = 1.0f - 2.0f * (x2 + y2);
#pragma unroll
        for (int i = 0; i < 3; ++i)
#pragma unroll
            for (int j = 0; j < 3; ++j) M[i * 3 + j] = Rq[i * 3 + j] * sc[j];
    };
    float cov[6];
    {
        float Rq[9], M[9];
        rot_and_m(Rq, M);
        cov[0] = M[0] * M[0] + M[1] * M[1] + M[2] * M[2];
        cov[1] = M[0] * M[3] + M[1] * M[4] + M[2] * M[5];
        cov[2] = M[0] * M[6] + M[1] * M[7] + M[2] * M[8];
        cov[3] = M[3] * M[3] + M[4] * M[4] + M[5] * M[5];
        cov[4] = M[3] * M[6] + M[4] * M[7] + M[5] * M[8];
        cov[5] = M[6] * M[6] + M[7] * M[7] + M[8] * M[8];
        asm volatile("" : "+v"(cov[0]), "+v"(cov[1]), "+v"(cov[2]), "+v"(cov[3]), "+v"(cov[4]), "+v"(cov[5]));
    }

    float v_mean[3] = {0, 0, 0};
    float vSw[6] = {0, 0, 0, 0, 0, 0};
    float v_k[12];
#pragma unroll
    for (int i = 0; i < 12; ++i) v_k[i] = 0.f;
    float v_opac = 0.f;

    for (int c = 0; c < C; ++c) {
        const int64_t pid = (int64_t)c * N + g;
        float4 g0, g1, g2;
        if (GATHER) {
            const int lane = threadIdx.x & 63, wv = threadIdx.x >> 6;
            float* wval = sVal + wv * (64 * ROW);
            const int my_end = cum[pid];
            const int my_start = !valid ? my_end : (pid == 0 ? 0 : cum[pid - 1]);
            const int s0 = __builtin_amdgcn_readfirstlane(my_start);
            const int s1 = __builtin_amdgcn_readlane(my_end, 63);
            float acc[ACC_VALS];
            float2 q0, q1, q2, q3, q4;
            auto fetch = [&](int u) {
                q0 = q1 = q2 = q3 = q4 = make_float2(0.f, 0.f);
                if (u < s1 && (unsigned)u < vt_cap) {
                    const float2* src = reinterpret_cast<const float2*>(vtile + (int64_t)u * VT_STRIDE);
                    q0 = src[0]; q1 = src[1]; q2 = src[2]; q3 = src[3]; q4 = src[4];
                }
            };
            auto rows_to_lds = [&]() {
                const bool live = __float_as_int(q4.y) == stamp;
                float* row = wval + lane * ROW;
                row[0] = live ? q0.x : 0.f; row[1] = live ? q0.y : 0.f; row[2] = live ? q1.x : 0.f;
                row[3] = live ? q1.y : 0.f; row[4] = live ? q2.x : 0.f; row[5] = live ? q2.y : 0.f;
                row[6] = live ? q3.x : 0.f; row[7] = live ? q3.y : 0.f; row[8] = live ? q4.x : 0.f;
            };
            if (s1 - s0 <= 64 * GATHER_WIDE_ABOVE) {
                if (s1 > s0) fetch(s0 + lane);
#pragma unroll
                for (int k2 = 0; k2 < ACC_VALS; ++k2) acc[k2] = 0.f;
                for (int base = s0; base < s1; base += 64) {
                    rows_to_lds();
                    wave_lds_sync();
                    fetch(base + 64 + lane);
                    const int lo = max(my_start, base) - base, hi = min(my_end, base + 64) - base;
                    for (int r = lo; r < hi; ++r) {
                        const float* src = wval + r * ROW;
#pragma unroll
                        for (int k2 = 0; k2 < ACC_VALS; ++k2) acc[k2] += src[k2];
                    }
                    wave_lds_sync();
                }
            } else {
                float* wacc = sAcc + wv * (64 * ROW);
                int* wst = sStart + wv * 65;
                wst[lane] = my_start;
                if (lane == 63) wst[64] = my_end;
#pragma unroll
                for (int k2 = 0; k2 < ACC_VALS; ++k2) wacc[lane * ROW + k2] = 0.f;
                const uint64_t tmask = touch ? __builtin_amdgcn_ballot_w64(valid && touch[pid] == (uint32_t)stamp) : ~0ull;
                auto meets = [&](int b) {
                    return __builtin_amdgcn_ballot_w64(my_end > my_start && my_start < b + 64 && my_end > b);
                };
                uint64_t pm_next = meets(s0);
                bool have = false;
                if (pm_next & tmask) { fetch(s0 + lane); have = true; }
                for (int base = s0; base < s1; base += 64) {
                    const uint64_t pm = pm_next & tmask;
                    const bool cur = have;
                    if (cur) { rows_to_lds(); wave_lds_sync(); }
                    pm_next = base + 64 < s1 ? meets(base + 64) : 0ull;
                    have = (pm_next & tmask) != 0;
                    if (have) fetch(base + 64 + lane);
                    if (cur) {
                        const int pa = __builtin_ctzll(pm), pb = 63 - __builtin_clzll(pm);
                        const int items = (pb - pa + 1) * ROW;
                        for (int it = lane; it < items; it += 64) {
                            const int q = (it * 7282) >> 16;
                            const int k2 = it - q * ROW, pp = pa + q;
                            const int lo = max(wst[pp], base) - base, hi = min(wst[pp + 1], base + 64) - base;
                            if (hi > lo) {
                                float sum = wacc[pp * ROW + k2];
                                const float* src = wval + k2;
                                int r = lo;
                                for (; r + 4 <= hi; r += 4) {
                                    const float a0 = src[r * ROW], a1 = src[(r + 1) * ROW], a2 = src[(r + 2) * ROW], a3 = src[(r + 3) * ROW];
                                    sum += a0; sum += a1; sum += a2; sum += a3;
                                }
                                for (; r < hi; ++r) sum += src[r * ROW];
                                wacc[pp * ROW + k2] = sum;
                            }
                        }
                        wave_lds_sync();
                    }
                }
                wave_lds_sync();
#pragma unroll
                for (int k2 = 0; k2 < ACC_VALS; ++k2) acc[k2] = wacc[lane * ROW + k2];
                wave_lds_sync();
            }
            g0 = make_float4(acc[0], acc[1], acc[2], acc[3]);
            g1 = make_float4(acc[4], acc[5], acc[6], acc[7]);
            g2 = make_float4(acc[8], 0.f, 0.f, 0.f);
            if (!valid) continue;
        }
        const float4 r2 = splats[pid * 3 + 2];
        if (__float_as_int(r2.z) <= 0) continue;
        const float4 r0 = splats[pid * 3 + 0];
        const float4 r1 = splats[pid * 3 + 1];
        if (!GATHER) {
            g0 = v_splats[pid * 3 + 0];
            g1 = v_splats[pid * 3 + 1];
            g2 = v_splats[pid * 3 + 2];
        }
        const float* o = cam + c * CAM_STRIDE;
        const float R[9] = {o[0], o[1], o[2], o[4], o[5], o[6], o[8], o[9], o[10]};
        v_opac += g0.z;
        {
            float dx = mx - o[20], dy = my - o[21], dz = mz - o[22];
            float nrm = sqrtf(dx * dx + dy * dy + dz * dz);
            float inrm = 1.0f / nrm;
            float ux = dx * inrm, uy = dy * inrm, uz = dz * inrm;
            const float vcol[3] = {g1.z, g1.w, g2.x};
            const float colf[3] = {r1.z, r1.w, r2.x};
            float vdx = 0.f, vdy = 0.f, vdz = 0.f;
#pragma unroll
            for (int ch = 0; ch < 3; ++ch) {
                float pre = SH_C0 * k[ch] + SH_C1 * ((-uy * k[3 + ch] + uz * k[6 + ch]) - ux * k[9 + ch]) + 0.5f;
                float vc = (colf[ch] > 0.0f || pre >= 0.0f) ? vcol[ch] : 0.0f;
                v_k[ch] += SH_C0 * vc;
                v_k[3 + ch] += -SH_C1 * uy * vc;
                v_k[6 + ch] += SH_C1 * uz * vc;
                v_k[9 + ch] += -SH_C1 * ux * vc;
                vdx += -SH_C1 * k[9 + ch] * vc;
                vdy += -SH_C1 * k[3 + ch] * vc;
                vdz += SH_C1 * k[6 + ch] * vc;
            }
            float dotp = vdx * ux + vdy * uy + vdz * uz;
            v_mean[0] += (vdx - dotp * ux) * inrm;
            v_mean[1] += (vdy - dotp * uy) * inrm;
            v_mean[2] += (vdz - dotp * uz) * inrm;
        }
        const float x = R[0] * mx + R[1] * my + R[2] * mz + o[3];
        const float y = R[3] * mx + R[4] * my + R[5] * mz + o[7];
        const float z = R[6] * mx + R[7] * my + R[8] * mz + o[11];
        float T[9];
#pragma unroll
        for (int i = 0; i < 3; ++i) {
            T[i * 3 + 0] = R[i * 3] * cov[0] + R[i * 3 + 1] * cov[1] + R[i * 3 + 2] * cov[2];
            T[i * 3 + 1] = R[i * 3] * cov[1] + R[i * 3 + 1] * cov[3] + R[i * 3 + 2] * cov[4];
            T[i * 3 + 2] = R[i * 3] * cov[2] + R[i * 3 + 1] * cov[4] + R[i * 3 + 2] * cov[5];
        }
        const float S00 = T[0] * R[0] + T[1] * R[1] + T[2] * R[2];
        const float S01 = T[0] * R[3] + T[1] * R[4] + T[2] * R[5];
        const float S02 = T[0] * R[6] + T[1] * R[7] + T[2] * R[8];
        const float S11 = T[3] * R[3] + T[4] * R[4] + T[5] * R[5];
        const float S12 = T[3] * R[6] + T[4] * R[7] + T[5] * R[8];
        const float S22 = T[6] * R[6] + T[7] * R[7] + T[8] * R[8];
        const float fx = o[12], fy = o[13];
        const float rz = 1.0f / z, rz2 = rz * rz, rz3 = rz2 * rz;
        const float xr = x * rz, yr = y * rz;
        const bool x_in = (xr <= o[16]) && (xr >= -o[17]);
        const bool y_in = (yr <= o[18]) && (yr >= -o[19]);
        const float tx = z * fminf(o[16], fmaxf(-o[17], xr));
        const float ty = z * fminf(o[18], fmaxf(-o[19], yr));
        const float a = fx * rz, cj = -fx * tx * rz2, b = fy * rz, d = -fy * ty * rz2;
        const Sym3 S = {S00, S01, S02, S11, S12, S22};
        Sym3 vS;
        float vJ00, vJ02, vJ11, vJ12;
        conic_chain(r0, r1, g0, g1, a, cj, b, d, S, vS, vJ00, vJ02, vJ11, vJ12);
        const float vm2x = g0.x, vm2y = g0.y;
        float vpx = fx * rz * vm2x;
        float vpy = fy * rz * vm2y;
        float vpz = -(fx * x * vm2x + fy * y * vm2y) * rz2;
        vpz += -fx * rz2 * vJ00 - fy * rz2 * vJ11;
        if (x_in) { vpx += -fx * rz2 * vJ02; vpz += 2.0f * fx * x * rz3 * vJ02; }
        else { vpz += fx * tx * rz3 * vJ02; }
        if (y_in) { vpy += -fy * rz2 * vJ12; vpz += 2.0f * fy * y * rz3 * vJ12; }
        else { vpz += fy * ty * rz3 * vJ12; }
        v_mean[0] += R[0] * vpx + R[3] * vpy + R[6] * vpz;
        v_mean[1] += R[1] * vpx + R[4] * vpy + R[7] * vpz;
        v_mean[2] += R[2] * vpx + R[5] * vpy + R[8] * vpz;
        float U[9];
        const float vSm[9] = {vS.xx, vS.xy, vS.xz, vS.xy, vS.yy, vS.yz, vS.xz, vS.yz, vS.zz};
#pragma unroll
        for (int i = 0; i < 3; ++i)
#pragma unroll
            for (int j = 0; j < 3; ++j)
                U[i * 3 + j] = vSm[i * 3] * R[j] + vSm[i * 3 + 1] * R[3 + j] + vSm[i * 3 + 2] * R[6 + j];
        vSw[0] += R[0] * U[0] + R[3] * U[3] + R[6] * U[6];
        vSw[1] += R[0] * U[1] + R[3] * U[4] + R[6] * U[7];
        vSw[2] += R[0] * U[2] + R[3] * U[5] + R[6] * U[8];
        vSw[3] += R[1] * U[1] + R[4] * U[4] + R[7] * U[7];
        vSw[4] += R[1] * U[2] + R[4] * U[5] + R[7] * U[8];
        vSw[5] += R[2] * U[2] + R[5] * U[5] + R[8] * U[8];
    }

    if (GATHER && !valid) return;
    float Rq[9], M[9];
    asm volatile("" : "+v"(qw), "+v"(qx), "+v"(qy), "+v"(qz));
    rot_and_m(Rq, M);
    const float W9[9] = {vSw[0], vSw[1], vSw[2], vSw[1], vSw[3], vSw[4], vSw[2], vSw[4], vSw[5]};
    float vM[9];
#pragma unroll
    for (int r = 0; r < 3; ++r)
#pragma unroll
        for (int s = 0; s < 3; ++s)
            vM[r * 3 + s] = 2.0f * (W9[r * 3] * M[s] + W9[r * 3 + 1] * M[3 + s] + W9[r * 3 + 2] * M[6 + s]);
    float v_scale[3], vR[9];
#pragma unroll
    for (int s = 0; s < 3; ++s) {
        v_scale[s] = Rq[s] * vM[s] + Rq[3 + s] * vM[3 + s] + Rq[6 + s] * vM[6 + s];
        vR[s] = vM[s] * sc[s]; vR[3 + s] = vM[3 + s] * sc[s]; vR[6 + s] = vM[6 + s] * sc[s];
    }
    float vq0 = 2.0f * (qx * (vR[7] - vR[5]) + qy * (vR[2] - vR[6]) + qz * (vR[3] - vR[1]));
    float vq1 = 2.0f * (-2.0f * qx * (vR[4] + vR[8]) + qy * (vR[3] + vR[1]) + qz * (vR[6] + vR[2]) + qw * (vR[7] - vR[5]));
    float vq2 = 2.0f * (qx * (vR[3] + vR[1]) - 2.0f * qy * (vR[0] + vR[8]) + qz * (vR[7] + vR[5]) + qw * (vR[2] - vR[6]));
    float vq3 = 2.0f * (qx * (vR[6] + vR[2]) + qy * (vR[7] + vR[5]) - 2.0f * qz * (vR[0] + vR[4]) + qw * (vR[3] - vR[1]));
    const float dq = vq0 * qw + vq1 * qx + vq2 * qy + vq3 * qz;
    vq0 = (vq0 - dq * qw) * inv_norm; vq1 = (vq1 - dq * qx) * inv_norm;
    vq2 = (vq2 - dq * qy) * inv_norm; vq3 = (vq3 - dq * qz) * inv_norm;

    const float sg = 1.0f / (1.0f + __expf(-opac));
    v_opac += reg_o_k * sg * (1.0f - sg);
    v_scale[0] += reg_s_k * __expf(s0);
    v_scale[1] += reg_s_k * __expf(s1);
    v_scale[2] += reg_s_k * __expf(s2);

    const int64_t Nl = range_major ? g_end - g_begin : N;
    float* gb = range_major ? grads + (int64_t)23 * g_begin : grads;
    const int gw = range_major ? g - g_begin : g;
    float* gm = gb; float* gq = gb + 3 * Nl; float* gs = gb + 7 * Nl;
    float* go = gb + 10 * Nl; float* gsh = gb + 11 * Nl;
    if (accumulate) {
        v_mean[0] += gm[3 * gw]; v_mean[1] += gm[3 * gw + 1]; v_mean[2] += gm[3 * gw + 2];
        vq0 += gq[4 * gw]; vq1 += gq[4 * gw + 1]; vq2 += gq[4 * gw + 2]; vq3 += gq[4 * gw + 3];
        v_scale[0] += gs[3 * gw]; v_scale[1] += gs[3 * gw + 1]; v_scale[2] += gs[3 * gw + 2];
        v_opac += go[gw];
#pragma unroll
        for (int i = 0; i < 12; ++i) v_k[i] += gsh[(int64_t)gw * 12 + i];
    }
    gm[3 * gw] = v_mean[0]; gm[3 * gw + 1] = v_mean[1]; gm[3 * gw + 2] = v_mean[2];
    gq[4 * gw] = vq0; gq[4 * gw + 1] = vq1; gq[4 * gw + 2] = vq2; gq[4 * gw + 3] = vq3;
    gs[3 * gw] = v_scale[0]; gs[3 * gw + 1] = v_scale[1]; gs[3 * gw + 2] = v_scale[2];
    go[gw] = v_opac;
#pragma unroll
    for (int i = 0; i < 12; ++i) gsh[(int64_t)gw * 12 + i] = v_k[i];
}

int st3r_project_sh_bwd_impl(hipStream_t s, const GsParams& g, const GsViews& v, float eps2d, const float* splats,
                             const float* v_splats, float reg_views, float opac_fac, float scale_fac, float* grads,
                             bool accumulate, int g_begin, int g_end, bool range_major, const st3r_vtile_ref* slots) {
    const int N = g.N, C = v.C;
    if (g_end < 0) g_end = N;
    if (N == 0 || g_end <= g_begin) return ST3R_OK;
    float reg_o_k = reg_views * opac_fac / (float)N;
    float reg_s_k = reg_views * scale_fac / (3.0f * (float)N);
    size_t shmem = (size_t)C * CAM_STRIDE * sizeof(float);
    if (slots)
        hipLaunchKernelGGL(k_project_sh_bwd<true>, dim3(ceil_div(g_end - g_begin, 256)), dim3(256), shmem, s, N, C, g.means,
                           g.quats, g.scales, g.opacities, g.sh, g.sh_stride, v.viewmats, v.Ks, v.campos, v.W, v.H, eps2d,
                           (const float4*)splats, (const float4*)nullptr, reg_o_k, reg_s_k, grads, accumulate ? 1 : 0, g_begin,
                           g_end, range_major ? 1 : 0, slots->cum, slots->vtile, slots->stamp, slots->vt_cap, slots->touch);
    else
        hipLaunchKernelGGL(k_project_sh_bwd<false>, dim3(ceil_div(g_end - g_begin, 256)), dim3(256), shmem, s, N, C, g.means,
                           g.quats, g.scales, g.opacities, g.sh, g.sh_stride, v.viewmats, v.Ks, v.campos, v.W, v.H, eps2d,
                           (const float4*)splats, (const float4*)v_splats, reg_o_k, reg_s_k, grads, accumulate ? 1 : 0, g_begin,
                           g_end, range_major ? 1 : 0, (const int32_t*)nullptr, (const float*)nullptr, 0, 0u, (const uint32_t*)nullptr);
    LAUNCH_CHECK();
    return ST3R_OK;
}

ST3R_EXPORT int st3r_gs_project_sh_bwd(st3r_ctx* ctx, void* stream, int N, int C, const float* means,
                                       const float* quats, const float* scales, const float* opacities,
                                       const float* sh, int sh_stride, const float* viewmats, const float* Ks,
                                       const float* campos, int width, int height, float eps2d,
                                       const float* splats, const float* v_splats, float reg_views,
                                       float opac_fac, float scale_fac, float* grads) {
    ARG_CHECK(ctx && N >= 0 && C > 0 && C <= ST3R_MAX_VIEWS && sh_stride >= 12);
    ARG_CHECK(means && quats && scales && opacities && sh && viewmats && Ks && campos && splats && v_splats && grads);
    return st3r_project_sh_bwd_impl((hipStream_t)stream, GsParams{N, means, quats, scales, opacities, sh, sh_stride},
                                    GsViews{C, width, height, viewmats, Ks, campos}, eps2d, splats, v_splats, reg_views, opac_fac, scale_fac,
                                    grads, false, 0, -1, false, nullptr);
}
```

starst3r_amd/csrc/project_common.h:

```cpp
#pragma once
#include <hip/hip_runtime.h>

#define SH_C0 0.2820947917738781f
#define SH_C1 0.48860251190292f

#define CAM_STRIDE 32

struct Sym3 { float xx, xy, xz, yy, yz, zz; };

__device__ __forceinline__ void conic_chain(const float4& r0, const float4& r1, const float4& g0, const float4& g1,
                                            const float& a, const float& cj, const float& b, const float& d,
                                            const Sym3& S, Sym3& vS, float& vJ00, float& vJ02, float& vJ11,
                                            float& vJ12) {
    const float A = r0.w, B = r1.x, Cc = r1.y;
    const float vA = g0.w, vB = 0.5f * g1.x, vC = g1.y;
    const float X00 = A * vA + B * vB, X01 = A * vB + B * vC;
    const float X10 = B * vA + Cc * vB, X11 = B * vB + Cc * vC;
    const float G00 = -(X00 * A + X01 * B);
    const float G01 = -0.5f * ((X00 * B + X01 * Cc) + (X10 * A + X11 * B));
    const float G11 = -(X10 * B + X11 * Cc);
    const float GJ00 = G00 * a, GJ01 = G01 * b, GJ02 = G00 * cj + G01 * d;
    const float GJ10 = G01 * a, GJ11 = G11 * b, GJ12 = G01 * cj + G11 * d;
    vS.xx = a * GJ00; vS.xy = a * GJ01; vS.xz = a * GJ02;
    vS.yy = b * GJ11; vS.yz = b * GJ12; vS.zz = cj * GJ02 + d * GJ12;
    vJ00 = 2.0f * (GJ00 * S.xx + GJ01 * S.xy + GJ02 * S.xz);
    vJ02 = 2.0f * (GJ00 * S.xz + GJ01 * S.yz + GJ02 * S.zz);
    vJ11 = 2.0f * (GJ10 * S.xy + GJ11 * S.yy + GJ12 * S.yz);
    vJ12 = 2.0f * (GJ10 * S.xz + GJ11 * S.yz + GJ12 * S.zz);
}
```

starst3r_amd/csrc/stages.h:

```cpp
#pragma once
#include "common.h"

struct GsParams {
    int N;
    const float *means, *quats, *scales, *opacities, *sh;
    int sh_stride;
};

struct GsViews {
    int C, W, H;
    const float *viewmats, *Ks, *campos;
    GsViews slice(int c0, int c1) const { return {c1 - c0, W, H, viewmats + 16 * c0, Ks + 9 * c0, campos + 3 * c0}; }
};

struct RasterOut {
    int C, W, H, tile_w, tile_h;
    const float* splats; const int32_t *offsets, *flat, *cum; const uint64_t *rects, *rectbase;
    int tight;
    int64_t n_pairs;
    int64_t n_isects, n_records, n_isects_ref, n_visible;
};

static inline RasterOut stage_lists(int C, int W, int H, int tile_w, int tile_h, const float* splats, const int32_t* offsets,
                                    const int32_t* flat, int64_t n_isects, const int32_t* cum = nullptr,
                                    int64_t n_pairs = 0) {
    return RasterOut{C, W, H, tile_w, tile_h, splats, offsets, flat, cum, nullptr, nullptr, 0, n_pairs, n_isects, n_isects,
                     n_isects, -1};
}

struct DepthPrior { const float* prior; const float* weight; const double* norm; float fac; };

struct ExposureReg { const float* exposure; float* v_exposure; };

struct LossWeight { const float* weight = nullptr; const double* norm = nullptr; int norm_stride = 0; int sums_stride = 2; };

struct Background { const float* colors; };

struct AlphaTarget { const float* target; const float* weight; const double* norm; float fac; };

int st3r_counts_buffer(st3r_ctx* ctx, hipStream_t s, int32_t** out);
int st3r_count_settle(st3r_ctx* ctx);
int st3r_train_fwd_bwd_impl(st3r_ctx* ctx, hipStream_t s, const GsParams& g, const GsViews& v, const float* gt_images,
                            float ssim_fac, float opac_fac, float scale_fac, float* grads, float* loss_out,
                            int64_t* stats_host, float* v_viewmats);
int st3r_peer_status_settle(st3r_ctx* ctx);

int st3r_project_impl(st3r_ctx* ctx, hipStream_t s, const GsParams& g, const GsViews& v, int tile_size, float eps2d,
                      float near_plane, float far_plane, float radius_clip, float* splats, int32_t* tiles_per_gauss,
                      double* reg_sums, uint64_t* depth_keys, int32_t* depth_vals, int tight, uint32_t key_base, void* rects,
                      int rect32, int reg_overwrite, double* zero_ptr, int zero_n, uint32_t* krange);
int st3r_project_sh_bwd_impl(hipStream_t s, const GsParams& g, const GsViews& v, float eps2d, const float* splats,
                             const float* v_splats, float reg_views, float opac_fac, float scale_fac, float* grads,
                             bool accumulate, int g_begin, int g_end, bool range_major, const st3r_vtile_ref* slots);

int st3r_isect_scan_impl(st3r_ctx* ctx, hipStream_t s, int64_t n_pairs, const int32_t* tiles, int32_t* cum,
                         int64_t* n_isects_host, const void* pack_rects, int rect32, uint64_t* pack_out,
                         int32_t** total_dev_out, int32_t* total_copy, int32_t* total_host);
int st3r_scan_tiles(int64_t n);
void st3r_emit_grid(int N, int C, int* bpc, int* grid, int* self_base);
void st3r_isect_constants(int64_t out[5]);
int st3r_isect_emit_chain_impl(st3r_ctx* ctx, hipStream_t s, int N, int C, const int32_t* perm, const void* rects,
                               int rect32, int tile_w, int tile_h, uint32_t* tile_keys, int32_t* vals, int64_t cap,
                               int band_tile, const int32_t* n_dev, const uint32_t** band_table);
int st3r_records_prepare_impl(hipStream_t s, int N, int C, const float* splats, int tile_size, int tile_w, int tile_h,
                              int tight, int32_t* tiles, uint64_t* depth_keys, int32_t* depth_vals, uint32_t key_base,
                              void* rects, int rect32);
int st3r_isect_offsets32_impl(hipStream_t s, int64_t n_isects, const uint32_t* keys, int C, int tile_w, int tile_h,
                              int32_t* offsets, const int32_t* n_dev);
int st3r_sort_tile_end_bit(int end_bit);
int st3r_sort_tile_impl(st3r_ctx* ctx, hipStream_t s, int64_t n, int end_bit, uint32_t* keys_in, int32_t* vals_in,
                        uint32_t* keys_out, int32_t* vals_out, const int32_t* n_dev);
int st3r_sort_tile_banded(int end_bit, int debug_flags);

int st3r_blend_fwd_impl(st3r_ctx* ctx, hipStream_t s, const RasterOut& ro, float* rgb, float* alpha, int32_t* last_ids,
                        bool for_backward, bool end_in_offsets);
int st3r_blend_fwd_cells_impl(st3r_ctx* ctx, hipStream_t s, const RasterOut& ro, float* rgb, float* alpha,
                              int32_t* last_ids, uint64_t* cmask, int64_t cmask_words, int32_t* tile_nb);
int st3r_blend_bwd_impl(st3r_ctx* ctx, hipStream_t s, const RasterOut& ro, const float* alpha, const int32_t* last_ids,
                        const float* v_rgb, const float* v_alpha, float* v_splats, bool end_in_offsets,
                        st3r_vtile_ref* defer);
int st3r_gather_vtile_impl(hipStream_t s, int64_t n_pairs, const st3r_vtile_ref* slots, float* v_splats);
int st3r_blend_depth_fwd_impl(st3r_ctx* ctx, hipStream_t s, const RasterOut& ro, const int32_t* last_ids, float* depth,
                              bool end_in_offsets);
int st3r_blend_depth_bwd_impl(st3r_ctx* ctx, hipStream_t s, const RasterOut& ro, const float* alpha,
                              const int32_t* last_ids, const float* v_depth, float* v_splats, bool end_in_offsets);
int st3r_add_pairs_impl(hipStream_t s, int64_t n_pairs, float* a, const float* b);

int st3r_loss_impl(st3r_ctx* ctx, hipStream_t s, int C, int H, int W, const float* render, const float* gt,
                   float w_l1, float w_ssim, double* sums, float* v_render, bool sums_cleared, const LossWeight& lw);
int st3r_loss_weight_for(st3r_ctx* ctx, hipStream_t s, const float* gt, int C, int H, int W, LossWeight* out);
int st3r_weight_norms(st3r_ctx* ctx, hipStream_t s, int C, int H, int W, const float* weight, double* out, int stride,
                      int at_least_one, bool interior, int slot);
int st3r_registered_weight_norms(st3r_ctx* ctx, hipStream_t s, const ViewReg& reg, const float* weight, int at_least_one,
                                 bool interior, int part_slot, int norm_slot, int* valid, const double** norms);
int st3r_depth_prior_for(st3r_ctx* ctx, hipStream_t s, const float* gt, int C, int H, int W, DepthPrior* out);
int st3r_depth_prior_loss_impl(st3r_ctx* ctx, hipStream_t s, int C, int H, int W, const float* depth, const float* alpha,
                               const float* prior, const float* weight, const double* norm, int norm_stride,
                               float depth_fac, double* sums, int sums_stride, float* v_depth, float* v_alpha);

void st3r_exposure_for(st3r_ctx* ctx, const float* gt, int C, int H, int W, ExposureReg* out);
int st3r_exposure_fwd_impl(hipStream_t s, int C, int H, int W, const float* rgb, const float* exposure, float* out);
int st3r_exposure_bwd_impl(st3r_ctx* ctx, hipStream_t s, int C, int H, int W, const float* rgb, const float* exposure,
                           const float* v_out, float* v_rgb, float* v_exposure);

void st3r_background_for(st3r_ctx* ctx, const float* gt, int C, int H, int W, Background* out);
int st3r_alpha_target_for(st3r_ctx* ctx, hipStream_t s, const float* gt, int C, int H, int W, AlphaTarget* out);
int st3r_composite_fwd_impl(hipStream_t s, int C, int H, int W, const float* rgb, const float* alpha,
                            const float* backgrounds, float* out);
int st3r_alpha_grad_impl(st3r_ctx* ctx, hipStream_t s, int C, int H, int W, const float* alpha, const float* backgrounds,
                         const float* v_out, const float* target, const float* weight, const double* norm, int norm_stride,
                         float alpha_fac, const float* v_alpha_in, double* sums, int sums_stride, float* v_alpha,
                         float* v_backgrounds);

float* st3r_intrinsics_grad_for(st3r_ctx* ctx, const float* gt, int C, int H, int W);

int st3r_adam_impl(hipStream_t s, int N, float* means, float* quats, float* scales, float* opacities, float* sh,
                   int sh_stride, const float* grads, float* m, float* v, double lr, double b1, double b2,
                   double eps, int step, const int32_t* count_dev, uint32_t count_cap, const int32_t* status_dev, int64_t i0,
                   int64_t i1, int64_t g0, int64_t g1, float* pstage, const float* gstage, float* grads_out);
int st3r_params_from_stage_impl(hipStream_t s, int N, float* means, float* quats, float* scales, float* opacities,
                                float* sh, int sh_stride, const float* pstage, int64_t i0, int64_t i1, int64_t lim,
                                const int32_t* count_dev, uint32_t count_cap, const int32_t* status_dev);
int st3r_params_from_peers_impl(hipStream_t s, int N, float* means, float* quats, float* scales, float* opacities,
                                float* sh, int sh_stride, const float* const* tab, int r, int64_t q, int64_t lim,
                                const int32_t* status_dev);
void st3r_adam_guard(st3r_ctx* ctx, const int32_t** count_dev, uint32_t* count_cap);
```

Baseline: 196.9.

## Recompute projection in backward instead of reading forward splat records

The projection backward kernel gains a RECORDS template flag. By default it now skips the per-view splat record reads (validity, conic, colour) and instead recomputes the conic and SH preactivation from the parameters. Views with no gathered gradient slots are skipped, and the colour clamp mask comes from the recomputed preactivation. Shared device helpers are factored out with contraction turned off so forward and backward stay bitwise consistent. Debug flags add a records path and forced range splitting with staging copies. The change trades global memory reads for extra ALU work and risks small gradient differences where the old mask used the stored colour.

```diff
diff --git a/starst3r_amd/build.py b/starst3r_amd/build.py
--- a/starst3r_amd/build.py
+++ b/starst3r_amd/build.py
@@ -14,6 +14,7 @@
 PER_FILE = {
     "gs_project.hip": ["-ffp-contract=off"],
     "gs_isect.hip": ["-ffp-contract=off"],
+    "gs_project_bwd.hip": ["-ffp-contract=off"],
     "recip_nn.hip": ["-mllvm", "-amdgpu-mfma-vgpr-form"],
 }
 NO_PACKED_F32 = ["-Xclang", "-target-feature", "-Xclang", "-packed-fp32-ops"]
diff --git a/starst3r_amd/csrc/fused_step.hip b/starst3r_amd/csrc/fused_step.hip
--- a/starst3r_amd/csrc/fused_step.hip
+++ b/starst3r_amd/csrc/fused_step.hip
@@ -312,18 +312,30 @@
                             const LossFacs& f, const float* v_pairs, const st3r_vtile_ref* slots, bool accumulate,
                             float* grads) {
     ctx->ranges_recorded = 0;
-    if (!(ctx->n_ranges > 1 && ctx->comm_stream))
+    const bool from_records = (ctx->debug_flags & 32768) != 0;
+    const int forced = (ctx->debug_flags & 65536) ? 2 : (ctx->debug_flags & 131072) ? 3 : 0;
+    const bool exchange = ctx->n_ranges > 1 && ctx->comm_stream;
+    if (!exchange && !forced)
         return st3r_project_sh_bwd_impl(s, g, v, 0.3f, ro.splats, v_pairs, (float)v.C, f.opac, f.scale, grads, accumulate, 0,
-                                        -1, false, slots);
+                                        -1, false, slots, from_records);
     ARENA_GET(SLOT_GSTAGE, float, (int64_t)23 * g.N, gstage);
-    const int K = ctx->n_ranges;
+    const int K = exchange ? ctx->n_ranges : forced;
     for (int j = 0; j < K; ++j) {
         const int g0 = (int)((int64_t)g.N * j / K), g1 = (int)((int64_t)g.N * (j + 1) / K);
         int rc = st3r_project_sh_bwd_impl(s, g, v, 0.3f, ro.splats, v_pairs, (float)v.C, f.opac, f.scale, gstage, accumulate,
-                                          g0, g1, true, slots);
+                                          g0, g1, true, slots, from_records);
         if (rc) return rc;
-        HIP_TRY(hipEventRecord(ctx->ev_range_bwd[j], s));
-    }
+        if (exchange) {
+            HIP_TRY(hipEventRecord(ctx->ev_range_bwd[j], s));
+            continue;
+        }
+        static const int off[5] = {0, 3, 7, 10, 11}, wid[5] = {3, 4, 3, 1, 12};
+        const int64_t Nl = g1 - g0;
+        for (int b = 0; b < 5 && Nl > 0; ++b)
+            HIP_TRY(hipMemcpyAsync(grads + (int64_t)off[b] * g.N + (int64_t)wid[b] * g0, gstage + (int64_t)23 * g0 + off[b] * Nl,
+                                   sizeof(float) * wid[b] * Nl, hipMemcpyDeviceToDevice, s));
+    }
+    if (!exchange) return ST3R_OK;
     ctx->ranges_recorded = K;
     return ST3R_OK;
 }
diff --git a/starst3r_amd/csrc/gs_intrinsics.hip b/starst3r_amd/csrc/gs_intrinsics.hip
--- a/starst3r_amd/csrc/gs_intrinsics.hip
+++ b/starst3r_amd/csrc/gs_intrinsics.hip
@@ -66,7 +66,7 @@
         const float a = fx * rz, cj = -fx * tx * rz2, b = fy * rz, d = -fy * ty * rz2;
         Sym3 vS;
         float vJ00, vJ02, vJ11, vJ12;
-        conic_chain(r0, r1, g0, g1, a, cj, b, d, S, vS, vJ00, vJ02, vJ11, vJ12);
+        conic_chain(r0.w, r1.x, r1.y, g0, g1, a, cj, b, d, S, vS, vJ00, vJ02, vJ11, vJ12);
         const float vm2x = g0.x, vm2y = g0.y;
         v_fx = vm2x * xr + vJ00 * rz;
         v_fy = vm2y * yr + vJ11 * rz;
diff --git a/starst3r_amd/csrc/gs_pose_bwd.hip b/starst3r_amd/csrc/gs_pose_bwd.hip
--- a/starst3r_amd/csrc/gs_pose_bwd.hip
+++ b/starst3r_amd/csrc/gs_pose_bwd.hip
@@ -108,7 +108,7 @@
         const Sym3 S = {S00, S01, S02, S11, S12, S22};
         Sym3 vS;
         float vJ00, vJ02, vJ11, vJ12;
-        conic_chain(r0, r1, g0, g1, a, cj, b, d, S, vS, vJ00, vJ02, vJ11, vJ12);
+        conic_chain(r0.w, r1.x, r1.y, g0, g1, a, cj, b, d, S, vS, vJ00, vJ02, vJ11, vJ12);
         const float vm2x = g0.x, vm2y = g0.y;
         float vpx = fx * rz * vm2x;
         float vpy = fy * rz * vm2y;
diff --git a/starst3r_amd/csrc/gs_project.hip b/starst3r_amd/csrc/gs_project.hip
--- a/starst3r_amd/csrc/gs_project.hip
+++ b/starst3r_amd/csrc/gs_project.hip
@@ -1,10 +1,6 @@
 #include "stages.h"
 #include "tile_rect.h"
 #include "project_common.h"
-
-__device__ __forceinline__ float dot3f(float a0, float a1, float a2, float b0, float b1, float b2) {
-    return (a0 * b0 + a1 * b1) + a2 * b2;
-}
 
 __global__ __launch_bounds__(256) void k_project_sh_fwd(
     int N, int C, const float* __restrict__ means, const float* __restrict__ quats,
@@ -18,19 +14,7 @@
     extern __shared__ float cam[];
     __shared__ float red[8];
     for (int c = threadIdx.x; c < C; c += blockDim.x) {
-        float* o = cam + c * CAM_STRIDE;
-        const float* V = viewmats + 16 * c;
-        for (int k = 0; k < 12; ++k) o[k] = V[k];
-        const float* K = Ks + 9 * c;
-        float fx = K[0], fy = K[4], cx = K[2], cy = K[5];
-        o[12] = fx; o[13] = fy; o[14] = cx; o[15] = cy;
-        float tan_fovx = 0.5f * (float)W / fx;
-        float tan_fovy = 0.5f * (float)H / fy;
-        o[16] = ((float)W - cx) / fx + 0.3f * tan_fovx;
-        o[17] = cx / fx + 0.3f * tan_fovx;
-        o[18] = ((float)H - cy) / fy + 0.3f * tan_fovy;
-        o[19] = cy / fy + 0.3f * tan_fovy;
-        o[20] = campos[3 * c]; o[21] = campos[3 * c + 1]; o[22] = campos[3 * c + 2];
+        cam_block_fill(cam + c * CAM_STRIDE, viewmats + 16 * c, Ks + 9 * c, campos + 3 * c, W, H);
     }
     __syncthreads();
 
@@ -48,21 +32,12 @@
         const float* kp = sh + (int64_t)g * sh_stride;
 #pragma unroll
         for (int i = 0; i < 12; ++i) k[i] = kp[i];
-        float n2 = ((qw * qw + qx * qx) + qy * qy) + qz * qz;
-        float inv = 1.0f / sqrtf(n2);
-        qw *= inv; qx *= inv; qy *= inv; qz *= inv;
-        float x2 = qx * qx, y2 = qy * qy, z2 = qz * qz;
-        float xy = qx * qy, xz = qx * qz, yz = qy * qz;
-        float wx = qw * qx, wy = qw * qy, wz = qw * qz;
-        float m0 = (1.0f - 2.0f * (y2 + z2)) * s0, m1 = (2.0f * (xy - wz)) * s1, m2 = (2.0f * (xz + wy)) * s2;
-        float m3 = (2.0f * (xy + wz)) * s0, m4 = (1.0f - 2.0f * (x2 + z2)) * s1, m5 = (2.0f * (yz - wx)) * s2;
-        float m6 = (2.0f * (xz - wy)) * s0, m7 = (2.0f * (yz + wx)) * s1, m8 = (1.0f - 2.0f * (x2 + y2)) * s2;
-        cov0 = dot3f(m0, m1, m2, m0, m1, m2);
-        cov1 = dot3f(m0, m1, m2, m3, m4, m5);
-        cov2 = dot3f(m0, m1, m2, m6, m7, m8);
-        cov3 = dot3f(m3, m4, m5, m3, m4, m5);
-        cov4 = dot3f(m3, m4, m5, m6, m7, m8);
-        cov5 = dot3f(m6, m7, m8, m6, m7, m8);
+        Quat q = {qw, qx, qy, qz};
+        float inv;
+        quat_normalize(q, inv);
+        Sym3 cw;
+        world_cov(q, s0, s1, s2, cw);
+        cov0 = cw.xx; cov1 = cw.xy; cov2 = cw.xz; cov3 = cw.yy; cov4 = cw.yz; cov5 = cw.zz;
         if (reg_part) {
             reg_o = 1.0f / (1.0f + __expf(-opac));
             reg_s = (__expf(s0) + __expf(s1)) + __expf(s2);
@@ -85,52 +60,26 @@
     uint32_t kmin = 0xFFFFFFFFu, kmax = 0u;
     for (int c = 0; active && c < C; ++c) {
         const float* o = cam + c * CAM_STRIDE;
-        const float R00 = o[0], R01 = o[1], R02 = o[2], t0 = o[3];
-        const float R10 = o[4], R11 = o[5], R12 = o[6], t1 = o[7];
-        const float R20 = o[8], R21 = o[9], R22 = o[10], t2 = o[11];
         const int64_t pid = (int64_t)c * N + g;
-        float x = dot3f(R00, R01, R02, mx, my, mz) + t0;
-        float y = dot3f(R10, R11, R12, mx, my, mz) + t1;
-        float z = dot3f(R20, R21, R22, mx, my, mz) + t2;
+        float x, y, z;
+        cam_point(o, mx, my, mz, x, y, z);
         bool valid = !(z < near_plane || z > far_plane);
         float m2x = 0, m2y = 0, ca = 0, cb = 0, cc = 0, radius = 0;
         if (valid) {
-            float T0 = dot3f(R00, R01, R02, cov0, cov1, cov2), T1 = dot3f(R00, R01, R02, cov1, cov3, cov4),
-                  T2 = dot3f(R00, R01, R02, cov2, cov4, cov5);
-            float T3 = dot3f(R10, R11, R12, cov0, cov1, cov2), T4 = dot3f(R10, R11, R12, cov1, cov3, cov4),
-                  T5 = dot3f(R10, R11, R12, cov2, cov4, cov5);
-            float T6 = dot3f(R20, R21, R22, cov0, cov1, cov2), T7 = dot3f(R20, R21, R22, cov1, cov3, cov4),
-                  T8 = dot3f(R20, R21, R22, cov2, cov4, cov5);
-            float c0 = dot3f(T0, T1, T2, R00, R01, R02);
-            float c1 = dot3f(T0, T1, T2, R10, R11, R12);
-            float c2 = dot3f(T0, T1, T2, R20, R21, R22);
-            float c3 = dot3f(T3, T4, T5, R10, R11, R12);
-            float c4 = dot3f(T3, T4, T5, R20, R21, R22);
-            float c5 = dot3f(T6, T7, T8, R20, R21, R22);
+            const Sym3 cw = {cov0, cov1, cov2, cov3, cov4, cov5};
+            Sym3 S;
+            cam_cov(o, cw, S);
             const float fx = o[12], fy = o[13], cx = o[14], cy = o[15];
-            float rz = 1.0f / z;
-            float rz2 = rz * rz;
-            float xr = x * rz, yr = y * rz;
-            float tx = z * fminf(o[16], fmaxf(-o[17], xr));
-            float ty = z * fminf(o[18], fmaxf(-o[19], yr));
-            float a = fx * rz, cj = -(fx * tx) * rz2;
-            float b = fy * rz, d = -(fy * ty) * rz2;
-            float t0x = a * c0 + cj * c2;
-            float t0y = a * c1 + cj * c4;
-            float t0z = a * c2 + cj * c5;
-            float t1y = b * c3 + d * c4;
-            float t1z = b * c4 + d * c5;
-            float c00 = t0x * a + t0z * cj;
-            float c01 = t0y * b + t0z * d;
-            float c11 = t1y * b + t1z * d;
+            ProjJ J;
+            proj_jacobian(o, x, y, z, J);
+            const float rz = J.rz;
+            float c00, c01, c11, det;
+            cov2d_of(S, J, eps2d, c00, c01, c11, det);
             m2x = (fx * x) * rz + cx;
             m2y = (fy * y) * rz + cy;
-            c00 += eps2d; c11 += eps2d;
-            float det = c00 * c11 - c01 * c01;
             if (det <= 0.0f) valid = false;
             else {
-                float inv_det = 1.0f / det;
-                ca = c11 * inv_det; cb = -c01 * inv_det; cc = c00 * inv_det;
+                conic_of(c00, c01, c11, det, ca, cb, cc);
                 float bb = 0.5f * (c00 + c11);
                 float v1 = bb + sqrtf(fmaxf(0.01f, bb * bb - det));
                 radius = ceilf(3.0f * sqrtf(v1));
@@ -144,15 +93,12 @@
         int ntiles = 0;
         TileRect tr = {0, 0, 0, 0};
         if (valid) {
-            float dx = mx - o[20], dy = my - o[21], dz = mz - o[22];
-            float inorm = 1.0f / sqrtf((dx * dx + dy * dy) + dz * dz);
-            dx *= inorm; dy *= inorm; dz *= inorm;
+            float ux, uy, uz, inorm;
+            view_dir(o, mx, my, mz, ux, uy, uz, inorm);
             float col[3];
 #pragma unroll
             for (int ch = 0; ch < 3; ++ch) {
-                float r = SH_C0 * k[ch];
-                r = r + SH_C1 * ((-dy * k[3 + ch] + dz * k[6 + ch]) - dx * k[9 + ch]);
-                r = r + 0.5f;
+                const float r = sh_pre(k[ch], k[3 + ch], k[6 + ch], k[9 + ch], ux, uy, uz);
                 col[ch] = r < 0.0f ? 0.0f : r;
             }
             tr = ref_tile_rect(m2x, m2y, radius, tile_size, tile_w, tile_h);
diff --git a/starst3r_amd/csrc/gs_project_bwd.hip b/starst3r_amd/csrc/gs_project_bwd.hip
--- a/starst3r_amd/csrc/gs_project_bwd.hip
+++ b/starst3r_amd/csrc/gs_project_bwd.hip
@@ -6,7 +6,7 @@
 #define GATHER_WIDE_ABOVE 6
 #endif
 
-template <bool GATHER>
+template <bool GATHER, bool RECORDS>
 __global__ __launch_bounds__(256) __attribute__((amdgpu_waves_per_eu(4))) void k_project_sh_bwd(
     int N, int C, const float* __restrict__ means, const float* __restrict__ quats,
     const float* __restrict__ scales, const float* __restrict__ opacities, const float* __restrict__ sh,
@@ -21,19 +21,7 @@
     __shared__ float sAcc[GATHER ? 256 * ROW : 1];
     __shared__ int sStart[GATHER ? 4 * 65 : 1];
     for (int c = threadIdx.x; c < C; c += blockDim.x) {
-        float* o = cam + c * CAM_STRIDE;
-        const float* V = viewmats + 16 * c;
-        for (int k = 0; k < 12; ++k) o[k] = V[k];
-        const float* K = Ks + 9 * c;
-        float fx = K[0], fy = K[4], cx = K[2], cy = K[5];
-        o[12] = fx; o[13] = fy; o[14] = cx; o[15] = cy;
-        float tan_fovx = 0.5f * (float)W / fx;
-        float tan_fovy = 0.5f * (float)H / fy;
-        o[16] = ((float)W - cx) / fx + 0.3f * tan_fovx;
-        o[17] = cx / fx + 0.3f * tan_fovx;
-        o[18] = ((float)H - cy) / fy + 0.3f * tan_fovy;
-        o[19] = cy / fy + 0.3f * tan_fovy;
-        o[20] = campos[3 * c]; o[21] = campos[3 * c + 1]; o[22] = campos[3 * c + 2];
+        cam_block_fill(cam + c * CAM_STRIDE, viewmats + 16 * c, Ks + 9 * c, campos + 3 * c, W, H);
     }
     __syncthreads();
     const int gbase = g_begin + blockIdx.x * blockDim.x;
@@ -49,8 +37,10 @@
     const float* kp = sh + (int64_t)g * sh_stride;
 #pragma unroll
     for (int i = 0; i < 12; ++i) k[i] = kp[i];
-    const float inv_norm = 1.0f / sqrtf(((qw * qw + qx * qx) + qy * qy) + qz * qz);
-    qw *= inv_norm; qx *= inv_norm; qy *= inv_norm; qz *= inv_norm;
+    float inv_norm;
+    Quat qn = {qw, qx, qy, qz};
+    quat_normalize(qn, inv_norm);
+    qw = qn.w; qx = qn.x; qy = qn.y; qz = qn.z;
     const float sc[3] = {s0, s1, s2};
     auto rot_and_m = [&](float (&Rq)[9], float (&M)[9]) {
         float x2 = qx * qx, y2 = qy * qy, z2 = qz * qz, xy = qx * qy, xz = qx * qz, yz = qy * qz;
@@ -63,18 +53,9 @@
 #pragma unroll
             for (int j = 0; j < 3; ++j) M[i * 3 + j] = Rq[i * 3 + j] * sc[j];
     };
-    float cov[6];
-    {
-        float Rq[9], M[9];
-        rot_and_m(Rq, M);
-        cov[0] = M[0] * M[0] + M[1] * M[1] + M[2] * M[2];
-        cov[1] = M[0] * M[3] + M[1] * M[4] + M[2] * M[5];
-        cov[2] = M[0] * M[6] + M[1] * M[7] + M[2] * M[8];
-        cov[3] = M[3] * M[3] + M[4] * M[4] + M[5] * M[5];
-        cov[4] = M[3] * M[6] + M[4] * M[7] + M[5] * M[8];
-        cov[5] = M[6] * M[6] + M[7] * M[7] + M[8] * M[8];
-        asm volatile("" : "+v"(cov[0]), "+v"(cov[1]), "+v"(cov[2]), "+v"(cov[3]), "+v"(cov[4]), "+v"(cov[5]));
-    }
+    Sym3 cov;
+    world_cov(qn, s0, s1, s2, cov);
+    asm volatile("" : "+v"(cov.xx), "+v"(cov.xy), "+v"(cov.xz), "+v"(cov.yy), "+v"(cov.yz), "+v"(cov.zz));
 
     float v_mean[3] = {0, 0, 0};
     float vSw[6] = {0, 0, 0, 0, 0, 0};
@@ -86,11 +67,13 @@
     for (int c = 0; c < C; ++c) {
         const int64_t pid = (int64_t)c * N + g;
         float4 g0, g1, g2;
+        bool has_slots = true;
         if (GATHER) {
             const int lane = threadIdx.x & 63, wv = threadIdx.x >> 6;
             float* wval = sVal + wv * (64 * ROW);
             const int my_end = cum[pid];
             const int my_start = !valid ? my_end : (pid == 0 ? 0 : cum[pid - 1]);
+            has_slots = my_end > my_start;
             const int s0 = __builtin_amdgcn_readfirstlane(my_start);
             const int s1 = __builtin_amdgcn_readlane(my_end, 63);
             float acc[ACC_VALS];
@@ -178,10 +161,11 @@
             g2 = make_float4(acc[8], 0.f, 0.f, 0.f);
             if (!valid) continue;
         }
-        const float4 r2 = splats[pid * 3 + 2];
-        if (__float_as_int(r2.z) <= 0) continue;
-        const float4 r0 = splats[pid * 3 + 0];
-        const float4 r1 = splats[pid * 3 + 1];
+        if (RECORDS) {
+            const float4 r2 = splats[pid * 3 + 2];
+            if (__float_as_int(r2.z) <= 0) continue;
+        } else if (!has_slots)
+            continue;
         if (!GATHER) {
             g0 = v_splats[pid * 3 + 0];
             g1 = v_splats[pid * 3 + 1];
@@ -191,17 +175,14 @@
         const float R[9] = {o[0], o[1], o[2], o[4], o[5], o[6], o[8], o[9], o[10]};
         v_opac += g0.z;
         {
-            float dx = mx - o[20], dy = my - o[21], dz = mz - o[22];
-            float nrm = sqrtf(dx * dx + dy * dy + dz * dz);
-            float inrm = 1.0f / nrm;
-            float ux = dx * inrm, uy = dy * inrm, uz = dz * inrm;
+            float ux, uy, uz, inrm;
+            view_dir(o, mx, my, mz, ux, uy, uz, inrm);
             const float vcol[3] = {g1.z, g1.w, g2.x};
-            const float colf[3] = {r1.z, r1.w, r2.x};
             float vdx = 0.f, vdy = 0.f, vdz = 0.f;
 #pragma unroll
             for (int ch = 0; ch < 3; ++ch) {
-                float pre = SH_C0 * k[ch] + SH_C1 * ((-uy * k[3 + ch] + uz * k[6 + ch]) - ux * k[9 + ch]) + 0.5f;
-                float vc = (colf[ch] > 0.0f || pre >= 0.0f) ? vcol[ch] : 0.0f;
+                const float pre = sh_pre(k[ch], k[3 + ch], k[6 + ch], k[9 + ch], ux, uy, uz);
+                float vc = pre >= 0.0f ? vcol[ch] : 0.0f;
                 v_k[ch] += SH_C0 * vc;
                 v_k[3 + ch] += -SH_C1 * uy * vc;
                 v_k[6 + ch] += SH_C1 * uz * vc;
@@ -215,34 +196,30 @@
             v_mean[1] += (vdy - dotp * uy) * inrm;
             v_mean[2] += (vdz - dotp * uz) * inrm;
         }
-        const float x = R[0] * mx + R[1] * my + R[2] * mz + o[3];
-        const float y = R[3] * mx + R[4] * my + R[5] * mz + o[7];
-        const float z = R[6] * mx + R[7] * my + R[8] * mz + o[11];
-        float T[9];
-#pragma unroll
-        for (int i = 0; i < 3; ++i) {
-            T[i * 3 + 0] = R[i * 3] * cov[0] + R[i * 3 + 1] * cov[1] + R[i * 3 + 2] * cov[2];
-            T[i * 3 + 1] = R[i * 3] * cov[1] + R[i * 3 + 1] * cov[3] + R[i * 3 + 2] * cov[4];
-            T[i * 3 + 2] = R[i * 3] * cov[2] + R[i * 3 + 1] * cov[4] + R[i * 3 + 2] * cov[5];
+        float x, y, z;
+        cam_point(o, mx, my, mz, x, y, z);
+        Sym3 S;
+        cam_cov(o, cov, S);
+        ProjJ J;
+        proj_jacobian(o, x, y, z, J);
+        const float fx = o[12], fy = o[13];
+        const float rz = J.rz, rz2 = J.rz2, rz3 = rz2 * rz;
+        const bool x_in = (J.xr <= o[16]) && (J.xr >= -o[17]);
+        const bool y_in = (J.yr <= o[18]) && (J.yr >= -o[19]);
+        const float tx = J.tx, ty = J.ty;
+        float cA, cB, cC;
+        if (RECORDS) {
+            const float4 r0 = splats[pid * 3 + 0];
+            const float4 r1 = splats[pid * 3 + 1];
+            cA = r0.w; cB = r1.x; cC = r1.y;
+        } else {
+            float c00, c01, c11, det;
+            cov2d_of(S, J, eps2d, c00, c01, c11, det);
+            conic_of(c00, c01, c11, det, cA, cB, cC);
         }
-        const float S00 = T[0] * R[0] + T[1] * R[1] + T[2] * R[2];
-        const float S01 = T[0] * R[3] + T[1] * R[4] + T[2] * R[5];
-        const float S02 = T[0] * R[6] + T[1] * R[7] + T[2] * R[8];
-        const float S11 = T[3] * R[3] + T[4] * R[4] + T[5] * R[5];
-        const float S12 = T[3] * R[6] + T[4] * R[7] + T[5] * R[8];
-        const float S22 = T[6] * R[6] + T[7] * R[7] + T[8] * R[8];
-        const float fx = o[12], fy = o[13];
-        const float rz = 1.0f / z, rz2 = rz * rz, rz3 = rz2 * rz;
-        const float xr = x * rz, yr = y * rz;
-        const bool x_in = (xr <= o[16]) && (xr >= -o[17]);
-        const bool y_in = (yr <= o[18]) && (yr >= -o[19]);
-        const float tx = z * fminf(o[16], fmaxf(-o[17], xr));
-        const float ty = z * fminf(o[18], fmaxf(-o[19], yr));
-        const float a = fx * rz, cj = -fx * tx * rz2, b = fy * rz, d = -fy * ty * rz2;
-        const Sym3 S = {S00, S01, S02, S11, S12, S22};
         Sym3 vS;
         float vJ00, vJ02, vJ11, vJ12;
-        conic_chain(r0, r1, g0, g1, a, cj, b, d, S, vS, vJ00, vJ02, vJ11, vJ12);
+        conic_chain(cA, cB, cC, g0, g1, J.a, J.cj, J.b, J.d, S, vS, vJ00, vJ02, vJ11, vJ12);
         const float vm2x = g0.x, vm2y = g0.y;
         float vpx = fx * rz * vm2x;
         float vpy = fy * rz * vm2y;
@@ -324,23 +301,27 @@
 
 int st3r_project_sh_bwd_impl(hipStream_t s, const GsParams& g, const GsViews& v, float eps2d, const float* splats,
                              const float* v_splats, float reg_views, float opac_fac, float scale_fac, float* grads,
-                             bool accumulate, int g_begin, int g_end, bool range_major, const st3r_vtile_ref* slots) {
+                             bool accumulate, int g_begin, int g_end, bool range_major, const st3r_vtile_ref* slots,
+                             bool from_records) {
     const int N = g.N, C = v.C;
     if (g_end < 0) g_end = N;
     if (N == 0 || g_end <= g_begin) return ST3R_OK;
     float reg_o_k = reg_views * opac_fac / (float)N;
     float reg_s_k = reg_views * scale_fac / (3.0f * (float)N);
     size_t shmem = (size_t)C * CAM_STRIDE * sizeof(float);
-    if (slots)
-        hipLaunchKernelGGL(k_project_sh_bwd<true>, dim3(ceil_div(g_end - g_begin, 256)), dim3(256), shmem, s, N, C, g.means,
-                           g.quats, g.scales, g.opacities, g.sh, g.sh_stride, v.viewmats, v.Ks, v.campos, v.W, v.H, eps2d,
-                           (const float4*)splats, (const float4*)nullptr, reg_o_k, reg_s_k, grads, accumulate ? 1 : 0, g_begin,
-                           g_end, range_major ? 1 : 0, slots->cum, slots->vtile, slots->stamp, slots->vt_cap, slots->touch);
+    const dim3 grid(ceil_div(g_end - g_begin, 256));
+#define PROJECT_BWD(GATHER, RECORDS, v_spl, ...)                                                                            \
+    hipLaunchKernelGGL((k_project_sh_bwd<GATHER, RECORDS>), grid, dim3(256), shmem, s, N, C, g.means, g.quats, g.scales,    \
+                       g.opacities, g.sh, g.sh_stride, v.viewmats, v.Ks, v.campos, v.W, v.H, eps2d, (const float4*)splats,  \
+                       (const float4*)(v_spl), reg_o_k, reg_s_k, grads, accumulate ? 1 : 0, g_begin, g_end,                 \
+                       range_major ? 1 : 0, __VA_ARGS__)
+    if (slots && !from_records)
+        PROJECT_BWD(true, false, nullptr, slots->cum, slots->vtile, slots->stamp, slots->vt_cap, slots->touch);
+    else if (slots)
+        PROJECT_BWD(true, true, nullptr, slots->cum, slots->vtile, slots->stamp, slots->vt_cap, slots->touch);
     else
-        hipLaunchKernelGGL(k_project_sh_bwd<false>, dim3(ceil_div(g_end - g_begin, 256)), dim3(256), shmem, s, N, C, g.means,
-                           g.quats, g.scales, g.opacities, g.sh, g.sh_stride, v.viewmats, v.Ks, v.campos, v.W, v.H, eps2d,
-                           (const float4*)splats, (const float4*)v_splats, reg_o_k, reg_s_k, grads, accumulate ? 1 : 0, g_begin,
-                           g_end, range_major ? 1 : 0, (const int32_t*)nullptr, (const float*)nullptr, 0, 0u, (const uint32_t*)nullptr);
+        PROJECT_BWD(false, true, v_splats, (const int32_t*)nullptr, (const float*)nullptr, 0, 0u, (const uint32_t*)nullptr);
+#undef PROJECT_BWD
     LAUNCH_CHECK();
     return ST3R_OK;
 }
@@ -355,5 +336,5 @@
     ARG_CHECK(means && quats && scales && opacities && sh && viewmats && Ks && campos && splats && v_splats && grads);
     return st3r_project_sh_bwd_impl((hipStream_t)stream, GsParams{N, means, quats, scales, opacities, sh, sh_stride},
                                     GsViews{C, width, height, viewmats, Ks, campos}, eps2d, splats, v_splats, reg_views, opac_fac, scale_fac,
-                                    grads, false, 0, -1, false, nullptr);
+                                    grads, false, 0, -1, false, nullptr, true);
 }
diff --git a/starst3r_amd/csrc/project_common.h b/starst3r_amd/csrc/project_common.h
--- a/starst3r_amd/csrc/project_common.h
+++ b/starst3r_amd/csrc/project_common.h
@@ -8,11 +8,131 @@
 
 struct Sym3 { float xx, xy, xz, yy, yz, zz; };
 
-__device__ __forceinline__ void conic_chain(const float4& r0, const float4& r1, const float4& g0, const float4& g1,
-                                            const float& a, const float& cj, const float& b, const float& d,
+__device__ __forceinline__ float dot3f(float a0, float a1, float a2, float b0, float b1, float b2) {
+#pragma clang fp contract(off)
+    return (a0 * b0 + a1 * b1) + a2 * b2;
+}
+
+__device__ __forceinline__ void cam_block_fill(float* o, const float* V, const float* K, const float* pos, int W, int H) {
+#pragma clang fp contract(off)
+    for (int k = 0; k < 12; ++k) o[k] = V[k];
+    float fx = K[0], fy = K[4], cx = K[2], cy = K[5];
+    o[12] = fx; o[13] = fy; o[14] = cx; o[15] = cy;
+    float tan_fovx = 0.5f * (float)W / fx;
+    float tan_fovy = 0.5f * (float)H / fy;
+    o[16] = ((float)W - cx) / fx + 0.3f * tan_fovx;
+    o[17] = cx / fx + 0.3f * tan_fovx;
+    o[18] = ((float)H - cy) / fy + 0.3f * tan_fovy;
+    o[19] = cy / fy + 0.3f * tan_fovy;
+    o[20] = pos[0]; o[21] = pos[1]; o[22] = pos[2];
+}
+
+struct Quat { float w, x, y, z; };
+
+__device__ __forceinline__ void quat_normalize(Quat& q, float& inv) {
+#pragma clang fp contract(off)
+    const float n2 = ((q.w * q.w + q.x * q.x) + q.y * q.y) + q.z * q.z;
+    inv = 1.0f / sqrtf(n2);
+    q.w *= inv; q.x *= inv; q.y *= inv; q.z *= inv;
+}
+
+__device__ __forceinline__ void world_cov(const Quat& q, const float& s0, const float& s1, const float& s2, Sym3& cov) {
+#pragma clang fp contract(off)
+    const float x2 = q.x * q.x, y2 = q.y * q.y, z2 = q.z * q.z;
+    const float xy = q.x * q.y, xz = q.x * q.z, yz = q.y * q.z;
+    const float wx = q.w * q.x, wy = q.w * q.y, wz = q.w * q.z;
+    const float m0 = (1.0f - 2.0f * (y2 + z2)) * s0, m1 = (2.0f * (xy - wz)) * s1, m2 = (2.0f * (xz + wy)) * s2;
+    const float m3 = (2.0f * (xy + wz)) * s0, m4 = (1.0f - 2.0f * (x2 + z2)) * s1, m5 = (2.0f * (yz - wx)) * s2;
+    const float m6 = (2.0f * (xz - wy)) * s0, m7 = (2.0f * (yz + wx)) * s1, m8 = (1.0f - 2.0f * (x2 + y2)) * s2;
+    cov.xx = dot3f(m0, m1, m2, m0, m1, m2);
+    cov.xy = dot3f(m0, m1, m2, m3, m4, m5);
+    cov.xz = dot3f(m0, m1, m2, m6, m7, m8);
+    cov.yy = dot3f(m3, m4, m5, m3, m4, m5);
+    cov.yz = dot3f(m3, m4, m5, m6, m7, m8);
+    cov.zz = dot3f(m6, m7, m8, m6, m7, m8);
+}
+
+__device__ __forceinline__ void cam_point(const float* o, const float& mx, const float& my, const float& mz, float& x,
+                                          float& y, float& z) {
+#pragma clang fp contract(off)
+    x = dot3f(o[0], o[1], o[2], mx, my, mz) + o[3];
+    y = dot3f(o[4], o[5], o[6], mx, my, mz) + o[7];
+    z = dot3f(o[8], o[9], o[10], mx, my, mz) + o[11];
+}
+
+__device__ __forceinline__ void cam_cov(const float* o, const Sym3& cov, Sym3& S) {
+#pragma clang fp contract(off)
+    const float R00 = o[0], R01 = o[1], R02 = o[2], R10 = o[4], R11 = o[5], R12 = o[6], R20 = o[8], R21 = o[9], R22 = o[10];
+    const float T0 = dot3f(R00, R01, R02, cov.xx, cov.xy, cov.xz), T1 = dot3f(R00, R01, R02, cov.xy, cov.yy, cov.yz),
+                T2 = dot3f(R00, R01, R02, cov.xz, cov.yz, cov.zz);
+    const float T3 = dot3f(R10, R11, R12, cov.xx, cov.xy, cov.xz), T4 = dot3f(R10, R11, R12, cov.xy, cov.yy, cov.yz),
+                T5 = dot3f(R10, R11, R12, cov.xz, cov.yz, cov.zz);
+    const float T6 = dot3f(R20, R21, R22, cov.xx, cov.xy, cov.xz), T7 = dot3f(R20, R21, R22, cov.xy, cov.yy, cov.yz),
+                T8 = dot3f(R20, R21, R22, cov.xz, cov.yz, cov.zz);
+    S.xx = dot3f(T0, T1, T2, R00, R01, R02);
+    S.xy = dot3f(T0, T1, T2, R10, R11, R12);
+    S.xz = dot3f(T0, T1, T2, R20, R21, R22);
+    S.yy = dot3f(T3, T4, T5, R10, R11, R12);
+    S.yz = dot3f(T3, T4, T5, R20, R21, R22);
+    S.zz = dot3f(T6, T7, T8, R20, R21, R22);
+}
+
+struct ProjJ { float rz, rz2, xr, yr, tx, ty, a, cj, b, d; };
+__device__ __forceinline__ void proj_jacobian(const float* o, const float& x, const float& y, const float& z, ProjJ& j) {
+#pragma clang fp contract(off)
+    const float fx = o[12], fy = o[13];
+    j.rz = 1.0f / z;
+    j.rz2 = j.rz * j.rz;
+    j.xr = x * j.rz; j.yr = y * j.rz;
+    j.tx = z * fminf(o[16], fmaxf(-o[17], j.xr));
+    j.ty = z * fminf(o[18], fmaxf(-o[19], j.yr));
+    j.a = fx * j.rz; j.cj = -(fx * j.tx) * j.rz2;
+    j.b = fy * j.rz; j.d = -(fy * j.ty) * j.rz2;
+}
+
+__device__ __forceinline__ void cov2d_of(const Sym3& S, const ProjJ& j, const float& eps2d, float& c00, float& c01,
+                                         float& c11, float& det) {
+#pragma clang fp contract(off)
+    const float t0x = j.a * S.xx + j.cj * S.xz;
+    const float t0y = j.a * S.xy + j.cj * S.yz;
+    const float t0z = j.a * S.xz + j.cj * S.zz;
+    const float t1y = j.b * S.yy + j.d * S.yz;
+    const float t1z = j.b * S.yz + j.d * S.zz;
+    c00 = t0x * j.a + t0z * j.cj;
+    c01 = t0y * j.b + t0z * j.d;
+    c11 = t1y * j.b + t1z * j.d;
+    c00 += eps2d; c11 += eps2d;
+    det = c00 * c11 - c01 * c01;
+}
+
+__device__ __forceinline__ void conic_of(const float& c00, const float& c01, const float& c11, const float& det,
+                                         float& ca, float& cb, float& cc) {
+#pragma clang fp contract(off)
+    const float inv_det = 1.0f / det;
+    ca = c11 * inv_det; cb = -c01 * inv_det; cc = c00 * inv_det;
+}
+
+__device__ __forceinline__ void view_dir(const float* o, const float& mx, const float& my, const float& mz, float& ux,
+                                         float& uy, float& uz, float& inorm) {
+#pragma clang fp contract(off)
+    ux = mx - o[20]; uy = my - o[21]; uz = mz - o[22];
+    inorm = 1.0f / sqrtf((ux * ux + uy * uy) + uz * uz);
+    ux *= inorm; uy *= inorm; uz *= inorm;
+}
+
+__device__ __forceinline__ float sh_pre(const float& k0, const float& k1, const float& k2, const float& k3,
+                                        const float& ux, const float& uy, const float& uz) {
+#pragma clang fp contract(off)
+    float r = SH_C0 * k0;
+    r = r + SH_C1 * ((-uy * k1 + uz * k2) - ux * k3);
+    r = r + 0.5f;
+    return r;
+}
+
+__device__ __forceinline__ void conic_chain(const float& A, const float& B, const float& Cc, const float4& g0,
+                                            const float4& g1, const float& a, const float& cj, const float& b, const float& d,
                                             const Sym3& S, Sym3& vS, float& vJ00, float& vJ02, float& vJ11,
                                             float& vJ12) {
-    const float A = r0.w, B = r1.x, Cc = r1.y;
     const float vA = g0.w, vB = 0.5f * g1.x, vC = g1.y;
     const float X00 = A * vA + B * vB, X01 = A * vB + B * vC;
     const float X10 = B * vA + Cc * vB, X11 = B * vB + Cc * vC;
diff --git a/starst3r_amd/csrc/stages.h b/starst3r_amd/csrc/stages.h
--- a/starst3r_amd/csrc/stages.h
+++ b/starst3r_amd/csrc/stages.h
@@ -51,7 +51,8 @@
                       int rect32, int reg_overwrite, double* zero_ptr, int zero_n, uint32_t* krange);
 int st3r_project_sh_bwd_impl(hipStream_t s, const GsParams& g, const GsViews& v, float eps2d, const float* splats,
                              const float* v_splats, float reg_views, float opac_fac, float scale_fac, float* grads,
-                             bool accumulate, int g_begin, int g_end, bool range_major, const st3r_vtile_ref* slots);
+                             bool accumulate, int g_begin, int g_end, bool range_major, const st3r_vtile_ref* slots,
+                             bool from_records);
 
 int st3r_isect_scan_impl(st3r_ctx* ctx, hipStream_t s, int64_t n_pairs, const int32_t* tiles, int32_t* cum,
                          int64_t* n_isects_host, const void* pack_rects, int rect32, uint64_t* pack_out,
```

Measured after the change: 199.1, median of 6. 1.1% higher.
